# ming71/rotate-yolov3

Measured on AMD Instinct MI355X. Metric: images/sec fwd+bwd at 608^2 (train step, backend=hip), higher is better.
Workload: dtype bf16; 1 GPU; configs[3]: Darknet-53 train step (fwd + riou loss + bwd + grad all-reduce + SGD), bs=64/GPU 608x608, synthetic HRSC-shaped targets; global_batch=64, parallelism=dp1, gradients=250 MB fp32 in 4 flat buckets, fp32 on the wire

## Files before the change

### include/ryolo.h

```cpp
#ifndef RYOLO_H
#define RYOLO_H

#include <stddef.h>
#include <stdint.h>

#ifdef __cplusplus
extern "C" {
#endif

#define RYOLO_OK 0
#define RYOLO_EINVAL -1
#define RYOLO_ELAUNCH -2
#define RYOLO_ETOOBIG -3

#define RYOLO_RNMS_MAX_BOXES 262144

const char *ryolo_strerror(int code);
int ryolo_abi_version(void);
const char *ryolo_build_id(void);
int ryolo_set_tuning(const char *name, const char *value);

size_t ryolo_rnms_workspace_bytes(int n);
int ryolo_rnms(const float *dets, int n, int row_stride, float thr, int64_t *keep_out, int32_t *num_keep,
               void *workspace, size_t workspace_bytes, void *stream);
// ... 49 lines not shown
#define RYOLO_CONV_KERNEL_STEM_DGRAD 7
#define RYOLO_CONV_KERNEL_STEM64 11
#define RYOLO_CONV_KERNEL_MQ128 9
#define RYOLO_CONV_KERNEL_MQ64 10
#define RYOLO_CONV_KERNEL_IGEMM 16
int ryolo_conv_kernel_choice(const ryolo_conv_desc *desc, int with_residual, int with_statistics);
#define RYOLO_WGRAD_KERNEL_TAPS 1000
int ryolo_conv_dgrad_kernel_choice(const ryolo_conv_desc *forward_desc, int with_bn_reduce );
int ryolo_conv_wgrad_kernel_choice(const ryolo_conv_desc *forward_desc);
int ryolo_nchw_f32_to_nhwc_bf16(const float *x, int N, int C, int H, int W, int Cpad, void *y, void *stream);
int ryolo_nhwc_bf16_to_nchw_f32(const void *x, int N, int C, int H, int W, int cstride, float *y, void *stream);


int ryolo_yolo_decode_filter(const void *head, int head_cstride, int bs, int ny, int nx, int na, int no,
                             const float *anchors, float stride, float context_factor, int arc, float conf_thres,
                             float min_wh, long long io_rows_per_image, long long io_row_offset, float *cand,
                             long long *cand_row, int *counter, int capacity, void *stream);

int ryolo_yolo_decode(const void *head, int head_cstride, int bs, int ny, int nx, int na, int no,
                      const float *anchors, float stride, float context_factor, int arc, float *io,
                      long long io_rows_per_image, long long io_row_offset, float *p, void *stream);

int ryolo_conv_head_decode_supported(const ryolo_conv_desc *desc, int na, int no);
int ryolo_conv_head_decode(const ryolo_conv_desc *desc, const void *x, const void *w_packed, const float *scale, const float *shift,
                           const float *anchors, int na, int no, float stride, float context_factor, int arc, float *io,
                           long long io_rows_per_image, long long io_row_offset, float *p, void *stream);

int ryolo_add_nhwc(const void *a, int a_cstride, const void *b, int b_cstride, void *y, int y_cstride,
                   long long npix, int C, void *stream);
int ryolo_upsample_nhwc(const void *x, int x_cstride, void *y, int y_cstride, int N, int H, int W, int C, int scale,
                        void *stream);
int ryolo_maxpool_nhwc(const void *x, int x_cstride, void *y, int y_cstride, int N, int H, int W, int C, int ksize,
                       int stride, void *stream);


int ryolo_conv0_recompute_supported(const ryolo_conv_desc *desc);
int ryolo_conv0_bn_act_fwd(const ryolo_conv_desc *desc, const void *x, const void *w_packed, const float *scale, const float *shift,
                           int act, const float *slope, void *y, void *stream);
size_t ryolo_conv0_bn_bwd_workspace_bytes(void);
int ryolo_conv0_bn_bwd(const ryolo_conv_desc *desc, const void *x, const void *w_packed, const void *dy, int dy_cstride,
                       const float *scale, const float *shift, const float *mean, const float *invstd, int act, const float *slope,
                       void *dz, int dz_cstride, float *dgamma, float *dbeta, float *dslope, void *workspace, size_t workspace_bytes,
                       int workspace_is_zero, void *stream);
size_t ryolo_conv0_bn_bwd_wgrad_workspace_bytes(void);
int ryolo_conv0_bn_bwd_wgrad(const ryolo_conv_desc *desc, const void *x, const void *w_packed, const void *dy, int dy_cstride,
                             const float *scale, const float *shift, const float *mean, const float *invstd, int act, const float *slope,
                             float *dgamma, float *dbeta, float *dslope, float *grad_oihw, int cin_real, int accumulate, void *workspace,
                             size_t workspace_bytes, void *stream);
int ryolo_conv_stat_rows(const ryolo_conv_desc *desc);
int ryolo_conv2d_bn_act_stats(const ryolo_conv_desc *desc, const void *x, const void *w_packed, const float *scale,
                              const float *shift, const void *residual, void *y,
                              double *stat_part ,
                              void *stream);
int ryolo_bn_finalize(double *stat_part, int rows, int cpad, int C, long long count, float eps, float momentum,
                      const float *gamma, const float *beta, float *mean, float *invstd, float *scale, float *shift,
                      float *running_mean , float *running_var, void *stream);
int ryolo_bn_act_fwd(const void *z, int z_cstride, const float *scale, const float *shift, int act,
                     const float *slope , const void *residual, int res_cstride, void *y,
                     int y_cstride, long long npix, int C, void *stream);
size_t ryolo_bn_act_bwd_workspace_bytes(long long npix, int C);
int ryolo_bn_act_bwd(const void *z, int z_cstride, const void *dy, int dy_cstride, const float *scale, const float *shift,
                     const float *mean, const float *invstd, int act, const float *slope, void *dz, int dz_cstride,
                     long long npix, int C, float *dgamma, float *dbeta, float *dslope, void *workspace,
                     size_t workspace_bytes, void *stream);
size_t ryolo_conv_packed_dgrad_bytes(int Cout, int Cin, int ksize, int stride);
int ryolo_conv_dgrad_tap_table(int ksize, int stride, int *host_out );
int ryolo_conv_pack_weights_dgrad(const float *w_oihw, int Cout, int Cin, int ksize, int stride, void *packed,
                                  const int *taps_table ,
                                  void *stream);
int ryolo_conv2d_dgrad(const ryolo_conv_desc *forward_desc, const void *dz, int dz_cstride, const void *packed_dgrad,
                       const float *ones, const float *zeros , void *dx, int accumulate, void *stream);
int ryolo_conv2d_dgrad_bnreduce_rows(const ryolo_conv_desc *forward_desc);
int ryolo_conv2d_dgrad_bnreduce(const ryolo_conv_desc *forward_desc, const void *dz, int dz_cstride, const void *packed_dgrad,
                                const float *ones, const float *zeros, void *dx, int accumulate,
                                const void *z , int z_cstride,
                                const float *scale, const float *shift, const float *mean, const float *invstd ,
                                const float *slope , float *part , void *stream);
int ryolo_bn_act_bwd_reduced(const void *z, int z_cstride, const void *dy, int dy_cstride, const float *scale, const float *shift,
                             const float *mean, const float *invstd, int act , const float *slope, void *dz,
                             int dz_cstride, long long npix, int C, float *dgamma, float *dbeta, float *dslope, const float *part,
                             int rows, void *workspace , size_t workspace_bytes, void *stream);
size_t ryolo_conv_wgrad_workspace_bytes(const ryolo_conv_desc *forward_desc);
int ryolo_conv2d_wgrad_partials(const ryolo_conv_desc *forward_desc, const void *x, const void *dz, int dz_cstride, int Cin_real,
                                float *grad_oihw, int accumulate, void *workspace, size_t workspace_bytes, void *stream);
int ryolo_conv2d_wgrad_reduce(const ryolo_conv_desc *forward_desc, const void *x, const void *dz, int dz_cstride, int Cin_real,
                              float *grad_oihw, int accumulate, void *workspace, size_t workspace_bytes, void *stream);

typedef struct ryolo_wgrad_reduce_job {
    const float *part;
    float *g;
    int S, Cout, Cin_real, Cin_k, ks, Kpad, Cout_pad, accumulate;
    int kind;
    int block_begin, block_end;
    int wide;
} ryolo_wgrad_reduce_job;
int ryolo_conv_wgrad_reduce_job_fill(ryolo_wgrad_reduce_job *host_job, const ryolo_conv_desc *forward_desc, int Cin_real, const void *workspace,
                                     float *grad_oihw, int accumulate);
int ryolo_conv_wgrad_reduce_batch(const ryolo_wgrad_reduce_job *device_jobs, int njobs, int total_blocks, void *stream);
int ryolo_conv2d_wgrad(const ryolo_conv_desc *forward_desc, const void *x, const void *dz, int dz_cstride, int Cin_real,
                       float *grad_oihw , int accumulate, void *workspace,
                       size_t workspace_bytes, void *stream);
int ryolo_upsample2x_bwd(const void *dy, int dy_cstride, void *dx, int dx_cstride, int N, int H, int W, int C,
                         int accumulate, void *stream);
int ryolo_pgrad_to_nhwc(const float *pgrad, int bs, int na, int ny, int nx, int no, void *out, int out_cstride,
                        void *stream);

typedef struct ryolo_pack_job {
    const void *src;
    void *dst;
    int kind, Cout, Cin, KS, Cin_pad, ntaps, Kpad, rows;
    int khs[9], kws[9];
    int block_begin, block_end;
// ... 57 lines not shown
```

### rotate-yolov3_amd/csrc/conv.hip

```cpp
#include <cstring>

#include <mutex>

#include "conv_common.h"

namespace ryolo_detail {
thread_local int *g_conv_choice = nullptr;
}

using namespace ryolo_detail;

namespace {

template <int KS, int BM, int BN, int WGM, int WGN, int NSTAGE, bool FAST, bool GEN, bool BNRED = false>
__global__ void __launch_bounds__(WGM *WGN * 64) conv_igemm_kernel(const ConvParams p, const BnRed br = BnRed()) {
    constexpr int NW = WGM * WGN, NT = NW * 64;
    constexpr int WPIX = BM / WGM, WCH = BN / WGN, PF = WPIX / 16, CF = WCH / 16;
    constexpr int A_BYTES = BM * BK * 2, B_BYTES = BN * BK * 2, STAGE = A_BYTES + B_BYTES;
    constexpr int A_PPW = (BM / 8) / NW, B_PPW = (BN / 8) / NW;
    static_assert(A_PPW >= 1 && B_PPW >= 1, "tile too small for the wave count");
    constexpr int SROW = BN * 2 + 16;
    static_assert(BM * SROW + WGM * 2 * BN * 4 <= NSTAGE * STAGE, "staging tile + statistics slots must fit in the operand buffers");
    constexpr int LOADS_PER_STAGE = A_PPW + B_PPW;

// ... 269 lines not shown
            const f32x4 sh = *(const f32x4 *)(p.shift + n0 + ch_local);
#pragma unroll
            for (int f = 0; f < PF; f++) {
                const int pix_local = wm * WPIX + f * 16 + frow;
                bf16x4 o;
#pragma unroll
                for (int r = 0; r < 4; r++) o[r] = (__bf16)actfn(acc[c][f][r] * sc[r] + sh[r]);
                *(bf16x4 *)(smem + pix_local * SROW + ch_local * 2) = o;
                if (GEN && p.stat_part) {
#pragma unroll
                    for (int r = 0; r < 4; r++) {
                        const float v = (float)o[r];
                        st_sum[c][r] += v;
                        st_sq[c][r] += v * v;
                    }
                }
            }
        }
    };
    const float slope = p.slope;
    if (p.act == RYOLO_ACT_LEAKY) epilogue1([slope](float v) { return v > 0.f ? v : v * slope; });
    else if (p.act == RYOLO_ACT_MISH) epilogue1([](float v) { return mish(v); });
    else epilogue1([](float v) { return v; });
    if (GEN && p.stat_part) {
        static_assert(CF <= 4, "one total per lane of a 16-lane row");
        float ta = 0.f, tb = 0.f;
#pragma unroll
        for (int c = 0; c < CF; c++)
#pragma unroll
            for (int r = 0; r < 4; r++) {
                const float a = row16_sum(st_sum[c][r]), b = row16_sum(st_sq[c][r]);
                if (frow == c * 4 + r) {
                    ta = a;
                    tb = b;
                }
            }
        float *slot = (float *)(smem + BM * SROW) + wm * 2 * BN;
        const int ch = wn * WCH + (frow >> 2) * 16 + fk * 4 + (frow & 3);
        if (frow < CF * 4) {
            slot[ch] = ta;
            slot[BN + ch] = tb;
        }
    }
    __syncthreads();
    if (GEN && p.stat_part) {
        static_assert(NT >= 2 * BN, "one thread per (statistic, channel)");
        if (tid < 2 * BN) {
            const float *slot = (const float *)(smem + BM * SROW);
            float v = slot[tid];
#pragma unroll
            for (int w = 1; w < WGM; w++) v += slot[w * 2 * BN + tid];
            const int st = tid / BN, ch = tid % BN;
            if (n0 + ch < p.Cout)
                atomicAdd(p.stat_part + (size_t)(m_tile % STAT_ROWS) * 2 * p.stat_cpad + (size_t)st * p.stat_cpad + n0 + ch, (double)v);
        }
    }

    constexpr int CPR = BN / 8;
    constexpr int NIT = BM * CPR / NT;
    static_assert(BM * CPR % NT == 0, "tile chunks must divide evenly over the threads");
    auto opix = [&](int m) -> size_t {
        int j, i, img;
        split_pixel(m, p.Wo, p.Ho, p.magic_wo, p.magic_ho, p.use_magic, j, i, img);
        return ((size_t)img * p.OH + (size_t)(i * p.os + p.ooy)) * p.OW + (size_t)(j * p.osx + p.oox);
    };
    bf16x8 rv[NIT];
    if (p.res) {
#pragma unroll
        for (int it = 0; it < NIT; it++) {
            const int idx = it * NT + tid;
            const int m = m0 + idx / CPR, c = n0 + (idx % CPR) * 8;
            const bool ok = (m < p.M) && (c < p.Cout);
            rv[it] = *(const bf16x8 *)(ok ? p.res + ((!GEN || p.os == 1) ? (size_t)m : opix(m)) * p.res_cs + c : zero_page);
        }
    }
    static_assert(!BNRED || (NT % CPR == 0 && CPR <= 16 && !GEN && CPR == BR_CPR && NIT == BR_NIT), "a thread keeps one 8-channel chunk for all its pixels");
    float bn_sc[8], bn_sh[8], bn_mu[8], bn_is[8], bs1[8], bs2[8], bs3[8];
    float bn_slope = 0.f;
    if constexpr (BNRED) {
        bn_slope = br.slope[0];
        const int c = n0 + (tid % CPR) * 8;
        const bool okc = c < p.Cout;
        const f32x4 z4 = f32x4{0.f, 0.f, 0.f, 0.f};
        const f32x4 a0 = okc ? *(const f32x4 *)(br.scale + c) : z4, a1 = okc ? *(const f32x4 *)(br.scale + c + 4) : z4;
        const f32x4 b0 = okc ? *(const f32x4 *)(br.shift + c) : z4, b1 = okc ? *(const f32x4 *)(br.shift + c + 4) : z4;
        const f32x4 u0 = okc ? *(const f32x4 *)(br.mean + c) : z4, u1 = okc ? *(const f32x4 *)(br.mean + c + 4) : z4;
        const f32x4 i0 = okc ? *(const f32x4 *)(br.invstd + c) : z4, i1 = okc ? *(const f32x4 *)(br.invstd + c + 4) : z4;
#pragma unroll
        for (int e = 0; e < 4; e++) {
            bn_sc[e] = a0[e]; bn_sc[4 + e] = a1[e]; bn_sh[e] = b0[e]; bn_sh[4 + e] = b1[e]; bn_mu[e] = u0[e]; bn_mu[4 + e] = u1[e];
            bn_is[e] = i0[e]; bn_is[4 + e] = i1[e];
        }
#pragma unroll
        for (int e = 0; e < 8; e++) bs1[e] = bs2[e] = bs3[e] = 0.f;
    }
#pragma unroll
    for (int it = 0; it < NIT; it++) {
        const int idx = it * NT + tid;
        const int pix = idx / CPR, ch = (idx % CPR) * 8;
        const int m = m0 + pix, c = n0 + ch;
        if (m >= p.M || c >= p.Cout) continue;
        bf16x8 v = *(const bf16x8 *)(smem + pix * SROW + ch * 2);
        if (p.res) {
#pragma unroll
            for (int e = 0; e < 8; e++) v[e] = (__bf16)((float)v[e] + (float)rv[it][e]);
        }
        if constexpr (BNRED) {
// ... 173 lines not shown

    const __bf16 *zero_page = p.w + (size_t)(((p.Cout + 127) >> 7) << 7) * p.Kpad;
    const int KT = p.Kpad / BK;
    const float slope = p.slope;
    f32x4 acc[CF][PF];

    int i = loc;
    setup(start + i);
    int m0 = nm0, n0 = nn0;
    int buf = 0;
    stage(0, buf, true);
    f32x4 ep_sc[CF], ep_sh[CF];
    auto load_scale_shift = [&]() {
#pragma unroll
        for (int c = 0; c < CF; c++) {
            const int ch_local = wn * WCH + c * 16 + fk * 4;
            ep_sc[c] = *(const f32x4 *)(p.scale + n0 + ch_local);
            ep_sh[c] = *(const f32x4 *)(p.shift + n0 + ch_local);
        }
    };
    load_scale_shift();
    float st_sum[CF][4], st_sq[CF][4];
#pragma unroll
    for (int c = 0; c < CF; c++)
#pragma unroll
        for (int r = 0; r < 4; r++) st_sum[c][r] = st_sq[c][r] = 0.f;
    auto flush_stats = [&]() {
        static_assert(!STATS || (CF <= 4 && NT >= 2 * BN), "one total per lane of a 16-lane row; one thread per (statistic, channel)");
        float ta = 0.f, tb = 0.f;
#pragma unroll
        for (int c = 0; c < CF; c++)
#pragma unroll
            for (int r = 0; r < 4; r++) {
                const float a = row16_sum(st_sum[c][r]), b = row16_sum(st_sq[c][r]);
                if (frow == c * 4 + r) {
                    ta = a;
                    tb = b;
                }
                st_sum[c][r] = st_sq[c][r] = 0.f;
            }
        float *slots = (float *)(smem + 2 * STAGE);
        const int ch = wn * WCH + (frow >> 2) * 16 + fk * 4 + (frow & 3);
        if (frow < CF * 4) {
            slots[wm * 2 * BN + ch] = ta;
            slots[wm * 2 * BN + BN + ch] = tb;
        }
        __syncthreads();
        if (tid < 2 * BN) {
            float v = slots[tid];
#pragma unroll
            for (int w = 1; w < WGM; w++) v += slots[w * 2 * BN + tid];
            const int st = tid / BN, c = tid % BN;
            if (n0 + c < p.Cout)
                atomicAdd(p.stat_part + ((size_t)(blockIdx.x % STAT_ROWS) * 2 + st) * p.stat_cpad + n0 + c, (double)v);
        }
        __syncthreads();
    };
    static_assert(!BNRED || (NT % CPR == 0 && CPR == 16 && !STATS), "a lane keeps one 8-channel chunk; 4 lanes of a wave share it");
    float bs1[8], bs2[8], bs3[8];
#pragma unroll
    for (int e = 0; e < 8; e++) bs1[e] = bs2[e] = bs3[e] = 0.f;
    const float bn_slope = BNRED ? br.slope[0] : 0.f;
    auto flush_bn = [&]() {
        if constexpr (BNRED) {
            const int cch = tid % CPR, c = n0 + cch * 8;
            float *slots = (float *)(smem + 2 * STAGE);
#pragma unroll
            for (int e = 0; e < 8; e++) {
                float a = bs1[e], b = bs2[e] * (c + e < p.Cout ? br.invstd[c + e] : 0.f), d = bs3[e];
                a += __shfl_xor(a, 16); b += __shfl_xor(b, 16); d += __shfl_xor(d, 16);
                a += __shfl_xor(a, 32); b += __shfl_xor(b, 32); d += __shfl_xor(d, 32);
                if (lane < CPR) {
                    slots[(wave * CPR + cch) * 24 + e] = a;
                    slots[(wave * CPR + cch) * 24 + 8 + e] = b;
                    slots[(wave * CPR + cch) * 24 + 16 + e] = d;
                }
                bs1[e] = bs2[e] = bs3[e] = 0.f;
            }
            __syncthreads();
            for (int t = tid; t < CPR * 24; t += NT) {
                const int l = t / 24, k = t % 24;
                float v = slots[l * 24 + k];
#pragma unroll
                for (int w = 1; w < NW; w++) v += slots[(w * CPR + l) * 24 + k];
                const int ch = n0 + l * 8 + (k & 7);
                if (ch < p.Cout) br.part[((size_t)blockIdx.x * 3 + (k >> 3)) * p.Cout + ch] += v;
            }
            __syncthreads();
        }
    };
    while (true) {
        const int inext = i + nloc;
        const bool has_next = inext < len;
#pragma unroll
        for (int c = 0; c < CF; c++)
#pragma unroll
            for (int f = 0; f < PF; f++) acc[c][f] = f32x4{0.f, 0.f, 0.f, 0.f};
        auto compute = [&](int cb) {
            const char *sb = smem + cb * STAGE;
#pragma unroll
            for (int ks = 0; ks < 2; ks++) {
                bf16x8 wf[CF], xf[PF];
#pragma unroll
                for (int c = 0; c < CF; c++) wf[c] = *(const bf16x8 *)(sb + b_off[c][ks]);
#pragma unroll
                for (int f = 0; f < PF; f++) xf[f] = *(const bf16x8 *)(sb + a_off[f][ks]);
#pragma unroll
// ... 324 lines not shown
    };
    u4 xa[3], xb[3];
    u2 da[2], db[2];
    request(xa, true);
    request_dy(da, m, true);
    for (int it = 0; it < n_it; it += 2) {
        const int m_a = m;
        advance();
        request(xb, it + 1 < n_it);
        request_dy(db, m, it + 1 < n_it);
        finish(xa, da, m_a, true);
        const int m_b = m;
        advance();
        request(xa, it + 2 < n_it);
        request_dy(da, m, it + 2 < n_it);
        finish(xb, db, m_b, it + 1 < n_it);
    }
    if constexpr (MODE == 2) {
        float t1 = 0.f, t2 = 0.f, t3 = 0.f;
#pragma unroll
        for (int cf = 0; cf < 2; cf++)
#pragma unroll
            for (int r = 0; r < 4; r++) {
                const float a1 = row16_sum(b1[cf][r]), a2 = row16_sum(b2[cf][r]), a3 = row16_sum(b3[cf][r]);
                if (fr == cf * 4 + r) {
                    t1 = a1;
                    t2 = a2;
                    t3 = a3;
                }
            }
        if (fr < 8) {
            const int ch = (fr >> 2) * 16 + g * 4 + (fr & 3);
            double *row = bw.part + (size_t)(wave_id % STAT_ROWS) * 3 * 32;
            atomicAdd(row + ch, (double)t1);
            atomicAdd(row + 32 + ch, (double)t2);
            atomicAdd(row + 64 + ch, (double)t3);
        }
        return;
    }
    if (STATS) {
        float ta = 0.f, tb = 0.f;
#pragma unroll
        for (int cf = 0; cf < 2; cf++)
#pragma unroll
            for (int r = 0; r < 4; r++) {
                const float a = row16_sum(st_sum[cf][r]), b = row16_sum(st_sq[cf][r]);
                if (fr == cf * 4 + r) {
                    ta = a;
                    tb = b;
                }
            }
        if (fr < 8) {
            const int ch = (fr >> 2) * 16 + g * 4 + (fr & 3);
            double *row = p.stat_part + (size_t)(wave_id % STAT_ROWS) * 2 * p.stat_cpad;
            atomicAdd(row + ch, (double)ta);
            atomicAdd(row + p.stat_cpad + ch, (double)tb);
        }
    }
}

__global__ void conv0_bwd_finalize_kernel(double *__restrict__ part, const float *__restrict__ scale, const float *__restrict__ mean,
                                          const float *__restrict__ invstd, float inv_count, float *__restrict__ kb, float *__restrict__ kd,
                                          float *__restrict__ dgamma, float *__restrict__ dbeta, float *__restrict__ dslope) {
    const int c = threadIdx.x;
    double a = 0.0, b = 0.0, d = 0.0;
    for (int r = 0; r < STAT_ROWS; r++) {
        double *row = part + (size_t)r * 96;
        a += row[c]; b += row[32 + c]; d += row[64 + c];
        row[c] = 0.0; row[32 + c] = 0.0; row[64 + c] = 0.0;
    }
    const float s1 = (float)a, s2 = (float)b * invstd[c];
    if (dgamma) dgamma[c] += s2;
    if (dbeta) dbeta[c] += s1;
    const float k = scale[c] * invstd[c] * s2 * inv_count;
    kb[c] = -k;
    kd[c] = k * mean[c] - scale[c] * s1 * inv_count;
    if (dslope) {
        float v = (float)d;
#pragma unroll
        for (int o = 16; o > 0; o >>= 1) v += __shfl_xor(v, o, 32);
        if (c == 0) dslope[0] += v;
    }
}

template <int ACT>
static int launch_c8_bwd(ConvParams &p, int gpw, unsigned nblk, const C8Bwd &bw, int mode, hipStream_t stream) {
    if (mode == 2) hipLaunchKernelGGL((conv3x3_c8_direct_kernel<false, ACT, 2>), dim3(nblk), dim3(256), 0, stream, p, gpw, bw);
    else hipLaunchKernelGGL((conv3x3_c8_direct_kernel<false, ACT, 3>), dim3(nblk), dim3(256), 0, stream, p, gpw, bw);
    return hipGetLastError() == hipSuccess ? RYOLO_OK : RYOLO_ELAUNCH;
}

template <bool STATS>
int launch_c8_direct(ConvParams &p, int gpw, unsigned nblk, hipStream_t stream) {
    if (STATS && p.y == nullptr) {
        hipLaunchKernelGGL((conv3x3_c8_direct_kernel<true, RYOLO_ACT_LINEAR, 1>), dim3(nblk), dim3(256), 0, stream, p, gpw, C8Bwd());
        return hipGetLastError() == hipSuccess ? RYOLO_OK : RYOLO_ELAUNCH;
    }
    if (p.act == RYOLO_ACT_LEAKY) hipLaunchKernelGGL((conv3x3_c8_direct_kernel<STATS, RYOLO_ACT_LEAKY>), dim3(nblk), dim3(256), 0, stream, p, gpw);
    else if (p.act == RYOLO_ACT_MISH) hipLaunchKernelGGL((conv3x3_c8_direct_kernel<STATS, RYOLO_ACT_MISH>), dim3(nblk), dim3(256), 0, stream, p, gpw);
    else hipLaunchKernelGGL((conv3x3_c8_direct_kernel<STATS, RYOLO_ACT_LINEAR>), dim3(nblk), dim3(256), 0, stream, p, gpw);
    return hipGetLastError() == hipSuccess ? RYOLO_OK : RYOLO_ELAUNCH;
}

__global__ void pack_weights_kernel(const float *__restrict__ w, int Cout, int Cin, int KS, int Cin_pad, int Kpad,
                                    int Cout_pad, __bf16 *__restrict__ out) {
    const size_t total = (size_t)Cout_pad * Kpad + 128;
    for (size_t i = (size_t)blockIdx.x * blockDim.x + threadIdx.x; i < total; i += (size_t)gridDim.x * blockDim.x) {
// ... 360 lines not shown
            if (pick == 1) pick = 7;
        }
    }
    if (pick == 8) return launch_conv_mp(p, 256, 0, stream);
    if (pick == 11) return launch_conv_mp(p, 192, 0, stream);
    if (pick == 14) return launch_conv_mp(p, 0, 0, stream);
    if (pick == 9) return launch_conv_mq(p, 0, stream);
#ifdef RYOLO_MP_ABLATION
    if (pick >= 32 && pick < 64) return launch_conv_mp(p, (pick & 16) ? 192 : 256, ryolo_mp_ablation_variant(pick & 15), stream);
    if (pick >= 64 && pick < 80) return launch_conv_mq(p, ryolo_mp_ablation_variant(pick & 15), stream);
#endif
    if (ksize == 1) {
        if (pick == 1) {
            const long long T = (((long long)p.M + 127) / 128) * ((p.Cout + 127) / 128);
            if (p.fast && p.os == 1 && !(p.stat_part && p.res) && !p.no_persist && (p.force_persist || 2 * T >= 5 * (long long)((2 * cu_count()) & ~7)))
                return launch_variant<1, 128, 128, 2, 2>(p, stream);
            p.no_persist = 1;
            return launch_variant<1, 128, 128, 2, 4>(p, stream);
        }
        if (pick == 7) return launch_variant<1, 128, 128, 2, 2>(p, stream);
        if (pick == 2) return launch_variant<1, 256, 64, 4, 1>(p, stream);
        if (pick == 3) return launch_variant<1, 256, 32, 4, 1>(p, stream);
        if (pick == 4) return launch_variant<1, 256, 128, 4, 2, 3>(p, stream);
        if (pick == 6) return launch_variant<1, 128, 128, 4, 2>(p, stream);
    } else {
        if (pick == 1) return launch_variant<3, 128, 128, 2, 4>(p, stream);
        if (pick == 7) return launch_variant<3, 128, 128, 2, 2>(p, stream);
        if (pick == 2) return launch_variant<3, 256, 64, 4, 1>(p, stream);
        if (pick == 3) return launch_variant<3, 256, 32, 4, 1>(p, stream);
        if (pick == 4) return launch_variant<3, 256, 128, 4, 2, 3>(p, stream);
        if (pick == 6) return launch_variant<3, 128, 128, 4, 2>(p, stream);
    }
    return RYOLO_EINVAL;
}

static int validate(const ryolo_conv_desc *d) {
    if (!d) return RYOLO_EINVAL;
    if (d->ksize != 1 && d->ksize != 3) return RYOLO_EINVAL;
    if (d->N <= 0 || d->H <= 0 || d->W <= 0 || d->Cin <= 0 || d->Cout <= 0 || d->stride <= 0) return RYOLO_EINVAL;
    if ((d->Cin & 7) || (d->Cout & 7) || (d->in_cstride & 7) || (d->out_cstride & 7)) return RYOLO_EINVAL;
    if (d->in_cstride < d->Cin || d->out_cstride < d->Cout) return RYOLO_EINVAL;
    if (d->upsample != 1 && d->upsample != 2) return RYOLO_EINVAL;
    if (d->ksize == 1 && d->pad != 0) return RYOLO_EINVAL;
    return RYOLO_OK;
}

int ryolo_conv_stat_rows(const ryolo_conv_desc *d) {
    if (validate(d) != RYOLO_OK) return 0;
    return STAT_ROWS;
}

int ryolo_conv2d_bn_act_stats(const ryolo_conv_desc *d, const void *x, const void *w_packed, const float *scale,
                              const float *shift, const void *residual, void *y, double *stat_part, void *stream_) {
    if (validate(d) != RYOLO_OK || !x || !w_packed || !scale || !shift) return RYOLO_EINVAL;
    if (!y && !(stat_part && ryolo_conv0_recompute_supported(d))) return RYOLO_EINVAL;
    if (residual && ((d->res_cstride & 7) || d->res_cstride < d->Cout)) return RYOLO_EINVAL;
    if (((uintptr_t)x | (uintptr_t)y | (uintptr_t)w_packed | (uintptr_t)residual | (uintptr_t)scale | (uintptr_t)shift) & 15)
        return RYOLO_EINVAL;
    ConvParams p;
    p.x = (const __bf16 *)x;
    p.w = (const __bf16 *)w_packed;
    p.scale = scale;
    p.shift = shift;
    p.res = (const __bf16 *)residual;
    p.y = (__bf16 *)y;
    p.N = d->N; p.H = d->H; p.W = d->W; p.Cin = d->Cin; p.in_cs = d->in_cstride;
    p.stride = d->stride;
    p.pad = d->pad;
    p.Ho = (d->H + 2 * d->pad - d->ksize) / d->stride + 1;
    p.Wo = (d->W + 2 * d->pad - d->ksize) / d->stride + 1;
    if (p.Ho <= 0 || p.Wo <= 0) return RYOLO_EINVAL;
    p.Cout = d->Cout; p.out_cs = d->out_cstride; p.res_cs = d->res_cstride;
    p.K = d->ksize * d->ksize * d->Cin;
    p.Kpad = (p.K + BK - 1) / BK * BK;
    const long long M = (long long)d->N * p.Ho * p.Wo;
    if (M > 0x7fffffffLL - 512) return RYOLO_EINVAL;
    p.M = (int)M;
    p.cin_log2 = ilog2_exact(d->Cin);
    if (d->ksize == 3 && p.cin_log2 < 0 && (d->Cin % BK)) return RYOLO_EINVAL;
    p.act = d->act; p.slope = d->slope; p.ups = d->upsample; p.nt = 0;
    {
        const unsigned long long xb = (((unsigned long long)d->N * d->H * d->W - 1) * d->in_cstride + d->Cin) * 2ull;
        const unsigned long long wb = ((unsigned long long)((d->Cout + 127) / 128 * 128) * p.Kpad + 128) * 2ull;
        p.taps2 = (d->Cin == 32 && d->ksize == 3) ? 1 : 0;
        p.fast = (d->Cin % BK == 0 || p.taps2) && xb < 0x7fffff00ull && wb < 0x7fffff00ull && !(d->tile & 0x100);
        if (!p.fast) p.taps2 = 0;
        p.x_bytes = (unsigned)(p.fast ? xb : 0);
        p.w_bytes = (unsigned)(p.fast ? wb : 0);
    }
    p.ntaps = d->ksize * d->ksize;
    for (int t = 0; t < 9; t++) { p.tap_dy[t] = t / d->ksize; p.tap_dx[t] = t % d->ksize; }
    p.os = 1; p.osx = 1; p.ooy = 0; p.oox = 0; p.OH = p.Ho; p.OW = p.Wo;
    p.no_persist = (d->tile & 0x200) ? 1 : 0;
    p.force_persist = (d->tile & 0x800) ? 1 : 0;
    p.pw_grid_cap = (d->tile & 0xff) == 13 ? (d->tile >> 16) & 0xff : 0;
#ifdef RYOLO_MP_ABLATION
    if ((d->tile & 0x400) && p.fast) p.x_bytes = p.w_bytes = 0;
#endif
    p.ntiles = 0; p.magic_wo = p.magic_ho = p.magic_nt = 0;
    p.nt_out = (long long)p.M * d->upsample * d->upsample * d->Cout * 2 >= nt_out_min_bytes() ? 1 : 0;
    p.stat_part = stat_part;
    p.stat_cpad = (d->Cout + 127) / 128 * 128;
    const unsigned long long c8_xb = (unsigned long long)d->N * d->H * d->W * 16ull, c8_yb = ((unsigned long long)(p.M - 1) * d->out_cstride + 32) * 2ull;
    if (d->ksize == 3 && d->stride == 1 && d->pad == 1 && d->Cin == 8 && d->in_cstride == 8 && d->Cout == 32 &&
        !residual && d->upsample == 1 && !(d->tile & 0x1ff) && p.Wo >= 16 && c8_xb < 0x7fffff00ull && c8_yb < 0x7fffff00ull) {
        p.x_bytes = (unsigned)c8_xb;
        p.w_bytes = (unsigned)c8_yb;
        const long long groups = ((long long)p.M + 15) / 16;
        const int gpw = (d->tile >> 16) ? (d->tile >> 16) : 32;
        const long long waves = (groups + gpw - 1) / gpw;
        const unsigned nblk = (unsigned)((waves + 3) / 4);
        const bool staged = conv0_halo_on() && !(d->tile >> 16) && y && !stat_part;
        RYOLO_CONV_DRY_RUN((staged ? RYOLO_CONV_KERNEL_STEM0 : RYOLO_CONV_KERNEL_DIRECT8));
        if (staged) return launch_conv0_halo(p, nullptr, 0, cu_count(), (hipStream_t)stream_);
        return stat_part ? launch_c8_direct<true>(p, gpw, nblk, (hipStream_t)stream_) : launch_c8_direct<false>(p, gpw, nblk, (hipStream_t)stream_);
    }
    return dispatch(p, d->ksize, pick_tile(d, d->Cout), (hipStream_t)stream_);
}

static bool head_params(const ryolo_conv_desc *d, ConvParams &p) {
    if (validate(d) != RYOLO_OK || d->ksize != 1 || d->stride != 1 || d->pad != 0 || d->upsample != 1 || (d->Cin % BK)) return false;
    p.N = d->N; p.H = d->H; p.W = d->W; p.Cin = d->Cin; p.in_cs = d->in_cstride; p.stride = 1; p.pad = 0; p.Ho = d->H; p.Wo = d->W;
    p.Cout = d->Cout; p.out_cs = d->Cout; p.res_cs = 0; p.K = d->Cin; p.Kpad = d->Cin;
    const long long M = (long long)d->N * d->H * d->W;
    if (M > 0x7fffffffLL - 512) return false;
    p.M = (int)M;
    p.act = d->act; p.slope = d->slope; p.ups = 1; p.nt = 0; p.taps2 = 0; p.os = 1; p.osx = 1; p.ooy = 0; p.oox = 0; p.OH = p.Ho; p.OW = p.Wo;
    const unsigned long long xb = (((unsigned long long)M - 1) * d->in_cstride + d->Cin) * 2ull;
    const unsigned long long wb = ((unsigned long long)((d->Cout + 127) / 128 * 128) * p.Kpad + 128) * 2ull;
    if (xb >= 0x7fffff00ull || wb >= 0x7fffff00ull) return false;
    p.fast = 1; p.x_bytes = (unsigned)xb; p.w_bytes = (unsigned)wb;
    p.res = nullptr; p.y = nullptr; p.stat_part = nullptr; p.stat_cpad = 0; p.nt_out = 0; p.pw_grid_cap = 0;
    p.no_persist = 0; p.force_persist = 0; p.ntaps = 1; p.ntiles = 0; p.magic_wo = p.magic_ho = p.magic_nt = 0; p.use_magic = 1;
    return true;
}

int ryolo_conv_head_decode_supported(const ryolo_conv_desc *d, int na, int no) {
    ConvParams p;
    return head_params(d, p) && conv_pw_decode_supported(p, na, no) ? 1 : 0;
}

int ryolo_conv_head_decode(const ryolo_conv_desc *d, const void *x, const void *w_packed, const float *scale, const float *shift,
                           const float *anchors, int na, int no, float stride, float context_factor, int arc, float *io,
                           long long io_rows_per_image, long long io_row_offset, float *pout, void *stream_) {
    ConvParams p;
    if (!x || !w_packed || !scale || !shift || !anchors || !io || !head_params(d, p) || !conv_pw_decode_supported(p, na, no)) return RYOLO_EINVAL;
    if (arc < 0 || arc > 2 || !(stride > 0.f) || !(context_factor > 0.f)) return RYOLO_EINVAL;
    if (((uintptr_t)x | (uintptr_t)w_packed) & 15) return RYOLO_EINVAL;
    p.x = (const __bf16 *)x; p.w = (const __bf16 *)w_packed; p.scale = scale; p.shift = shift;
    return launch_conv_pw_decode(p, io, io_rows_per_image, io_row_offset, pout, anchors, na, no, stride, context_factor, arc, (hipStream_t)stream_);
}

int ryolo_conv_pair_supported(const ryolo_conv_desc *first, const ryolo_conv_desc *second, int shortcut_from_input) {
    if (validate(first) != RYOLO_OK || validate(second) != RYOLO_OK) return 0;
    return conv_stem_pair_kind(first, second, shortcut_from_input) != 0 ? 1 : 0;
// ... 702 lines not shown
```

### rotate-yolov3_amd/csrc/conv_common.h

```cpp
#pragma once
#include <hip/hip_runtime.h>
#include <stdint.h>
#include <stdlib.h>

#include "../../include/ryolo.h"

namespace ryolo_detail {

typedef __attribute__((ext_vector_type(8))) __bf16 bf16x8;
typedef __attribute__((ext_vector_type(4))) __bf16 bf16x4;
typedef __attribute__((ext_vector_type(2))) __bf16 bf16x2;
typedef __attribute__((ext_vector_type(4))) float f32x4;
typedef __attribute__((ext_vector_type(4))) unsigned int u32x4;
typedef __attribute__((address_space(3))) void *lds_vp;
typedef const __attribute__((address_space(1))) void *glb_vp;

constexpr int BK = 64;
constexpr long long NT_OUT_MIN_BYTES = 128ll << 20;
constexpr int STAT_ROWS = 128;

struct ConvParams {
    const __bf16 *x;
    const __bf16 *w;
    const float *scale;
    const float *shift;
    const __bf16 *res;
    __bf16 *y;
    int N, H, W, Cin, in_cs;
    int Ho, Wo, Cout, out_cs, res_cs;
    int stride, pad;
    int K, Kpad, M;
    int cin_log2;
    int act;
    float slope;
    int ups;
    int nt;
    unsigned x_bytes, w_bytes;
    int fast;
    int taps2;
    int no_persist;
    int force_persist;
    int ntaps;
    int tap_dy[9], tap_dx[9];
    int os, ooy, oox, OH, OW;
    int osx;
    int ntiles;
    unsigned magic_wo, magic_ho, magic_nt;
    int use_magic;
    unsigned y_bytes, res_bytes;
    double *stat_part;
    int stat_cpad;
    int nt_out;
    int reg3;
    int korder = 0;
    int dbg0, dbg1;
    int pw_nb, pw_mb;
    unsigned *trace;
    int pw_grid_cap;
};

struct BnRed {
    const __bf16 *z;
    int z_cs;
    const float *scale, *shift, *mean, *invstd;
    const float *slope;
    float *part;
    unsigned z_bytes = 0;
};

__device__ __forceinline__ float mish(float v) {
    const float e = __expf(fminf(v, 20.f));
    const float n = (1.f + e) * (1.f + e);
    return v * (n - 1.f) / (n + 1.f);
}

__device__ __forceinline__ float row16_sum(float v) {
#if defined(__HIP_DEVICE_COMPILE__)
    v += __builtin_bit_cast(float, __builtin_amdgcn_update_dpp(0, __builtin_bit_cast(int, v), 0xB1, 0xF, 0xF, true));
    v += __builtin_bit_cast(float, __builtin_amdgcn_update_dpp(0, __builtin_bit_cast(int, v), 0x4E, 0xF, 0xF, true));
    v += __builtin_bit_cast(float, __builtin_amdgcn_update_dpp(0, __builtin_bit_cast(int, v), 0x141, 0xF, 0xF, true));
    v += __builtin_bit_cast(float, __builtin_amdgcn_update_dpp(0, __builtin_bit_cast(int, v), 0x140, 0xF, 0xF, true));
#endif
    return v;
}

template <int O>
__device__ __forceinline__ float lane_xor_sum(float v) {
#if defined(__HIP_DEVICE_COMPILE__)
    if constexpr (O == 4) {
        v += __builtin_bit_cast(float, __builtin_amdgcn_update_dpp(0, __builtin_bit_cast(int, v), 0x124, 0xF, 0xF, true));
    } else if constexpr (O == 8) {
        v += __builtin_bit_cast(float, __builtin_amdgcn_update_dpp(0, __builtin_bit_cast(int, v), 0x128, 0xF, 0xF, true));
    } else if constexpr (O == 16) {
        const unsigned u = __builtin_bit_cast(unsigned, v);
        const auto s = __builtin_amdgcn_permlane16_swap(u, u, false, false);
        v = __builtin_bit_cast(float, (unsigned)s[0]) + __builtin_bit_cast(float, (unsigned)s[1]);
    } else {
        static_assert(O == 32, "partner distance");
        const unsigned u = __builtin_bit_cast(unsigned, v);
        const auto s = __builtin_amdgcn_permlane32_swap(u, u, false, false);
        v = __builtin_bit_cast(float, (unsigned)s[0]) + __builtin_bit_cast(float, (unsigned)s[1]);
    }
#endif
    return v;
// ... 92 lines not shown
```

### rotate-yolov3_amd/csrc/conv_mp.hip

```cpp
#include <cstdlib>
#include <type_traits>

#include "conv_common.h"

using namespace ryolo_detail;

namespace {

constexpr int MP_BN = 256;
constexpr int MP_XB = 256 * 128, MP_WB = 256 * 128;
constexpr int MP_OPS = 2 * MP_XB + 2 * MP_WB;
constexpr int MP_SS = 2 * 2 * MP_BN * 4;
constexpr int MP_TRACE = 8 * 128 * 4;
constexpr int MP_LDS = MP_OPS + MP_SS + MP_TRACE;
constexpr int MP_STAT_NT = 4;
constexpr int MP_STAT = MP_STAT_NT * 2 * 2 * MP_BN * 4;
constexpr int MP_LDS_GEN = MP_LDS + MP_STAT;

template <int N> using ic = std::integral_constant<int, N>;

template <int BM, int GEN, int VAR, int KO = 0>
__global__ void __launch_bounds__(512) conv_mp_kernel(const ConvParams p) {
    constexpr int OPS = MP_OPS;
    constexpr int WBASE = 2 * MP_XB, XBASE = 0;
// ... 381 lines not shown
                    unsigned R[2][2];
#pragma unroll
                    for (int cc = 0; cc < 2; cc++) {
                        const int c = 2 * h + cc;
                        bf16x4 o;
#pragma unroll
                        for (int r = 0; r < 4; r++) {
                            float v = acc[c][f][r] * sc[cc][r] + sh[cc][r];
                            if constexpr (ACT == RYOLO_ACT_LEAKY) v = v > 0.f ? v : v * slope;
                            else if constexpr (ACT == 3) v = fmaxf(v, v * slope);
                            else if constexpr (ACT == RYOLO_ACT_MISH) v = mish(v);
                            o[r] = (__bf16)v;
                            if (GEN == 1 && p.stat_part && ok) {
                                const float q = (float)o[r];
                                st_sum[cc][r] += q;
                                st_sq[cc][r] += q * q;
                            }
                        }
                        const uint2 u = __builtin_bit_cast(uint2, o);
                        R[cc][0] = u.x;
                        R[cc][1] = u.y;
                    }
#if defined(__HIP_DEVICE_COMPILE__)
#pragma unroll
                    for (int d = 0; d < 2; d++) {
                        auto s1 = __builtin_amdgcn_permlane32_swap(R[0][d], R[1][d], false, false);
                        auto s2 = __builtin_amdgcn_permlane16_swap(s1[0], s1[1], false, false);
                        R[0][d] = s2[0];
                        R[1][d] = s2[1];
                    }
#endif
                    u32x4 out = u32x4{R[0][0], R[0][1], R[1][0], R[1][1]};
                    if (has_res) {
                        bf16x8 a = __builtin_bit_cast(bf16x8, out);
                        const bf16x8 b = __builtin_bit_cast(bf16x8, rv[f][h]);
#pragma unroll
                        for (int e = 0; e < 8; e++) a[e] = (__bf16)((float)a[e] + (float)b[e]);
                        out = __builtin_bit_cast(u32x4, a);
                    }
                    if constexpr (NO_STORE) {
                        asm volatile("" ::"v"(out.x), "v"(out.y), "v"(out.z), "v"(out.w));
                    } else {
                        int voff = yoff0, soff = f * ystep;
                        if (strided) { voff = (opix(ok ? m : 0) * p.out_cs + chq + fk * 8) * 2; soff = 0; }
                        voff = ok ? voff : (int)0x80000000;
#if defined(__HIP_DEVICE_COMPILE__)
                        if (STAUX == 0 && p.nt_out) buffer_store16_soff<2>(out, yrs, voff + 64 * h, soff);
                        else buffer_store16_soff<STAUX>(out, yrs, voff + 64 * h, soff);
#endif
                    }
                }
                stamp_e(3 + h);
                if (GEN == 1 && p.stat_part) {
                    double *row = p.stat_part + (size_t)(((m0 / BM) * 2 + wm) % STAT_ROWS) * 2 * p.stat_cpad;
                    float *slot = stat_lds + ((size_t)((n0 / MP_BN) * 2 + wm) * 2) * MP_BN + wn * 64;
                    float ta = 0.f, tb = 0.f;
#pragma unroll
                    for (int cc = 0; cc < 2; cc++)
#pragma unroll
                        for (int r = 0; r < 4; r++) {
                            const float a = row16_sum(st_sum[cc][r]), b = row16_sum(st_sq[cc][r]);
                            if (frow == cc * 4 + r) {
                                ta = a;
                                tb = b;
                            }
                        }
                    if (frow < 8) {
                        const int cl = (2 * h + (frow >> 2)) * 16 + fr4 + (frow & 3);
                        if (stat_in_lds) {
                            slot[cl] += ta;
                            slot[MP_BN + cl] += tb;
                        } else {
                            atomicAdd(row + chq + cl, (double)ta);
                            atomicAdd(row + p.stat_cpad + chq + cl, (double)tb);
                        }
                    }
                }
            }
          };
          if (p.act == RYOLO_ACT_LEAKY && p.slope <= 1.f) run_epilogue(ic<3>{});
          else if (p.act == RYOLO_ACT_LEAKY) run_epilogue(ic<RYOLO_ACT_LEAKY>{});
          else if (p.act == RYOLO_ACT_MISH) run_epilogue(ic<RYOLO_ACT_MISH>{});
          else run_epilogue(ic<RYOLO_ACT_LINEAR>{});
          ss[(sslot ^ 1) * (2 * MP_BN) + tid] = ss_next;
        }
        stamp_e(5);
        te_tile++;
        __builtin_amdgcn_sched_barrier(0);
        if (!has_next) break;
        sslot = __builtin_amdgcn_readfirstlane(sslot ^ 1);
        ti = tnext;
        m0 = nm0;
        n0 = nn0;
    }
    if constexpr (STAGGER) {
        if (wm == 0) __builtin_amdgcn_s_barrier();
    }
    if constexpr (GEN == 1) {
        if (stat_in_lds) {
            asm volatile("s_waitcnt lgkmcnt(0)" ::: "memory");
            __builtin_amdgcn_s_barrier();
            double *row = p.stat_part + (size_t)(blockIdx.x % STAT_ROWS) * 2 * p.stat_cpad;
            for (int i = tid; i < p.nt * 2 * MP_BN; i += 512) {
                const int s_ = i / (2 * MP_BN), st = (i / MP_BN) & 1, ch = i % MP_BN;
                const float *q = stat_lds + ((size_t)(s_ * 2) * 2 + st) * MP_BN + ch;
                const float v = q[0] + q[2 * MP_BN];
                if (v != 0.f && s_ * MP_BN + ch < p.Cout) atomicAdd(row + (size_t)st * p.stat_cpad + s_ * MP_BN + ch, (double)v);
            }
        }
    }
    asm volatile("s_waitcnt vmcnt(0)" ::: "memory");
    if constexpr (TRACE_EPI) {
        if ((blockIdx.x == 0 || blockIdx.x == 8 || blockIdx.x == 129) && p.stat_part) {
            asm volatile("s_waitcnt lgkmcnt(0)" ::: "memory");
            unsigned *dst = (unsigned *)p.stat_part + ((blockIdx.x == 0 ? 0 : (blockIdx.x == 8 ? 1 : 2)) * 8 + wave) * 32;
            if (lane < 32) dst[lane] = *(const unsigned *)(smem + trace_off + lane * 4);
        }
    }
}

inline unsigned mp_magic_u32(int d) { return d <= 1 ? 0u : (unsigned)((0x100000000ull + (unsigned)d - 1) / (unsigned)d); }

inline int mp_cu_count() {
    static int cus = 0;
    if (!cus) {
        int dev = 0;
        if (hipGetDevice(&dev) != hipSuccess ||
            hipDeviceGetAttribute(&cus, hipDeviceAttributeMultiprocessorCount, dev) != hipSuccess || cus <= 0)
            cus = 256;
    }
    return cus;
}

void *g_trace_buf = nullptr;
int g_dbg[4] = {0, 0, 0, 0};
int g_var[16] = {0};

template <int BM, int GEN, int VAR, int KO = 0>
int mp_launch(ConvParams &p, hipStream_t stream) {
    if (VAR & (128 | 1024)) p.stat_part = (double *)g_trace_buf;
    static bool attr_done = false;
    constexpr int LDS = GEN == 1 ? MP_LDS_GEN : MP_LDS;
    auto kfn = conv_mp_kernel<BM, GEN, VAR, KO>;
    if (!attr_done && !g_conv_choice) {
        if (hipFuncSetAttribute((const void *)kfn, hipFuncAttributeMaxDynamicSharedMemorySize, LDS) != hipSuccess)
            return RYOLO_ELAUNCH;
        attr_done = true;
    }
    const int mt = (p.M + BM - 1) / BM;
    p.nt = (p.Cout + MP_BN - 1) / MP_BN;
    const long long T = (long long)mt * p.nt;
    const long long dmax = p.Wo > p.Ho ? p.Wo : p.Ho, mpad = (long long)mt * BM;
    if (mpad * dmax >= 0x100000000ll || T * p.nt >= 0x100000000ll || T > 0x7fffffffll) return RYOLO_EINVAL;
    p.use_magic = 1;
    p.magic_wo = mp_magic_u32(p.Wo);
// ... 83 lines not shown
```

### rotate-yolov3_amd/csrc/conv_mq.hip

```cpp
#include <cstdlib>
#include <type_traits>

#include "conv_common.h"

using namespace ryolo_detail;

namespace {

#ifdef RYOLO_MP_ABLATION
constexpr int Q_TRACE = 4 * 128 * 4;
#else
constexpr int Q_TRACE = 0;
#endif
template <int CW, int PF>
struct QL {
    static constexpr int BN = 4 * CW;
    static constexpr int BM = 16 * PF;
    static constexpr int XB = BM * 128;
    static constexpr int WB = BN * 128;
    static constexpr int XBASE = 0, WBASE = 2 * XB;
    static constexpr int OPS = 2 * XB + WB;
    static constexpr int SS = 2 * 2 * BN * 4;
    static constexpr int LDS = OPS + SS + Q_TRACE;
    static constexpr int STAT_NT = CW == 64 ? 4 : 8;
// ... 431 lines not shown
                        auto s2 = __builtin_amdgcn_permlane16_swap(s1[0], s1[1], false, false);
                        R[0][d] = s2[0];
                        R[1][d] = s2[1];
                    }
#endif
                    u32x4 out = u32x4{R[0][0], R[0][1], R[1][0], R[1][1]};
                    if (has_res) {
                        bf16x8 a = __builtin_bit_cast(bf16x8, out);
                        const bf16x8 b = __builtin_bit_cast(bf16x8, rv[f][h]);
#pragma unroll
                        for (int e = 0; e < 8; e++) a[e] = (__bf16)((float)a[e] + (float)b[e]);
                        out = __builtin_bit_cast(u32x4, a);
                    }
                    if constexpr (BNRED) {
                        const bf16x8 a = __builtin_bit_cast(bf16x8, out), zb = __builtin_bit_cast(bf16x8, zv[f][h]);
#pragma unroll
                        for (int e = 0; e < 8; e++) {
                            const float zf = (float)zb[e], d = ok ? (float)a[e] : 0.f;
                            const float u = zf * bn_sc[e] + bn_sh[e];
                            float g = d;
                            if (u <= 0.f) { g = d * bn_slope; bs3[e] += d * u; }
                            bs2[e] += g * (zf - bn_mu[e]);
                            bs1[e] += g;
                        }
                    }
                    if constexpr (NO_STORE) {
                        asm volatile("" ::"v"(out.x), "v"(out.y), "v"(out.z), "v"(out.w));
                    } else {
                        int voff = yoff0, soff = f * ystep;
                        if (strided) { voff = (opix(ok ? m : 0) * p.out_cs + chq + fk * 8) * 2; soff = 0; }
                        voff = ok ? voff : (int)0x80000000;
#if defined(__HIP_DEVICE_COMPILE__)
                        if (p.nt_out) buffer_store16_soff<2>(out, yrs, voff + 64 * h, soff);
                        else buffer_store16_soff<0>(out, yrs, voff + 64 * h, soff);
#endif
                    }
                }
                stamp_e(3 + h);
                if constexpr (BNRED) {
                    float t1 = 0.f, t2 = 0.f, t3 = 0.f;
#pragma unroll
                    for (int e = 0; e < 8; e++) {
                        const float a = row16_sum(bs1[e]), b = row16_sum(bs2[e]), c = row16_sum(bs3[e]);
                        if (frow == e) { t1 = a; t2 = b; t3 = c; }
                    }
                    if (frow < 8) {
                        float *slot = stat_lds + (size_t)(n0 / Q_BN) * 3 * Q_BN + wn * CW + 32 * h + fk * 8 + frow;
                        slot[0] += t1;
                        slot[Q_BN] += t2;
                        slot[2 * Q_BN] += t3;
                    }
                }
                if (GEN == 1 && p.stat_part) {
                    double *row = p.stat_part + (size_t)((m0 / L::BM) % STAT_ROWS) * 2 * p.stat_cpad;
                    float *slot = stat_lds + (size_t)(n0 / Q_BN) * 2 * Q_BN + wn * CW;
                    float ta = 0.f, tb = 0.f;
#pragma unroll
                    for (int cc = 0; cc < 2; cc++)
#pragma unroll
                        for (int r = 0; r < 4; r++) {
                            const float a = row16_sum(st_sum[cc][r]), b = row16_sum(st_sq[cc][r]);
                            if (frow == cc * 4 + r) {
                                ta = a;
                                tb = b;
                            }
                        }
                    if (frow < 8) {
                        const int cl = (2 * h + (frow >> 2)) * 16 + fr4 + (frow & 3);
                        if (stat_in_lds) {
                            slot[cl] += ta;
                            slot[Q_BN + cl] += tb;
                        } else {
                            atomicAdd(row + chq + cl, (double)ta);
                            atomicAdd(row + p.stat_cpad + chq + cl, (double)tb);
                        }
                    }
                }
            }
          };
          if (p.act == RYOLO_ACT_LEAKY && p.slope <= 1.f) run_epilogue(ic<3>{});
          else if (p.act == RYOLO_ACT_LEAKY) run_epilogue(ic<RYOLO_ACT_LEAKY>{});
          else if (p.act == RYOLO_ACT_MISH) run_epilogue(ic<RYOLO_ACT_MISH>{});
          else run_epilogue(ic<RYOLO_ACT_LINEAR>{});
          ss[(sslot ^ 1) * (2 * Q_BN) + sst] = ssn0;
          ss[(sslot ^ 1) * (2 * Q_BN) + Q_BN + sst] = ssn1;
        }
        stamp_e(5);
        te_tile++;
        __builtin_amdgcn_sched_barrier(0);
        if (!has_next) break;
        sslot = __builtin_amdgcn_readfirstlane(sslot ^ 1);
        ti = tnext;
        m0 = nm0;
        n0 = nn0;
    }
    if constexpr (GEN == 1) {
        if (stat_in_lds) {
            asm volatile("s_waitcnt lgkmcnt(0)" ::: "memory");
            __builtin_amdgcn_s_barrier();
            double *row = p.stat_part + (size_t)(blockIdx.x % STAT_ROWS) * 2 * p.stat_cpad;
            for (int i = tid; i < p.nt * 2 * Q_BN; i += 256) {
                const int s_ = i / (2 * Q_BN), st = (i / Q_BN) & 1, ch = i % Q_BN;
                const float v = stat_lds[(size_t)(s_ * 2 + st) * Q_BN + ch];
                if (v != 0.f && s_ * Q_BN + ch < p.Cout) atomicAdd(row + (size_t)st * p.stat_cpad + s_ * Q_BN + ch, (double)v);
            }
        }
    }
    if constexpr (BNRED) {
        asm volatile("s_waitcnt lgkmcnt(0)" ::: "memory");
        __builtin_amdgcn_s_barrier();
        for (int i = tid; i < p.nt * 3 * Q_BN; i += 256) {
            const int s_ = i / (3 * Q_BN), k3 = (i / Q_BN) % 3, ch = s_ * Q_BN + i % Q_BN;
            if (ch < p.Cout) {
                float v = stat_lds[i];
                if (k3 == 1) v *= br.invstd[ch];
                br.part[((size_t)blockIdx.x * 3 + k3) * p.Cout + ch] = v;
            }
        }
    }
    asm volatile("s_waitcnt vmcnt(0)" ::: "memory");
    if constexpr (TRACE_EPI) {
        if ((blockIdx.x == 0 || blockIdx.x == 256 || blockIdx.x == 8) && p.stat_part) {
            asm volatile("s_waitcnt lgkmcnt(0)" ::: "memory");
            unsigned *dst = (unsigned *)p.stat_part + ((blockIdx.x == 0 ? 0 : (blockIdx.x == 256 ? 1 : 2)) * 8 + wn) * 32;
            if (lane < 32) dst[lane] = *(const unsigned *)(smem + trace_off + lane * 4);
        }
    }
}

inline unsigned mq_magic_u32(int d) { return d <= 1 ? 0u : (unsigned)((0x100000000ull + (unsigned)d - 1) / (unsigned)d); }

inline int mq_cu_count() {
    static int cus = 0;
    if (!cus) {
        int dev = 0;
        if (hipGetDevice(&dev) != hipSuccess ||
            hipDeviceGetAttribute(&cus, hipDeviceAttributeMultiprocessorCount, dev) != hipSuccess || cus <= 0)
            cus = 256;
    }
    return cus;
}

#ifdef RYOLO_MP_ABLATION
void *g_q_trace_buf = nullptr;
int g_q_dbg[4] = {0, 0, 0, 0};
#endif

inline int mq_grid_for(long long T, int cw = 64) {
    int per_cu = 2;
    if (cw == 32) {
        const char *e = abl_env("RYOLO_MQ128_WGPC");
        const int v = e ? atoi(e) : 2;
        if (v >= 1 && v <= 4) per_cu = v;
// ... 143 lines not shown
```

### rotate-yolov3_amd/csrc/conv_pw.hip

```cpp
#include <type_traits>
#include <utility>

#include "conv_common.h"
#include "yolo_decode.h"

using namespace ryolo_detail;

namespace {

template <int N> using ic = std::integral_constant<int, N>;

template <class F, int... I>
__device__ __forceinline__ void static_for_impl(F &&f, std::integer_sequence<int, I...>) {
    (f(ic<I>{}), ...);
}
template <int N, class F>
__device__ __forceinline__ void static_for(F &&f) {
    static_for_impl(f, std::make_integer_sequence<int, N>{});
}

__device__ __forceinline__ void issue_order_fence() { asm volatile("" ::: "memory"); }

template <int N>
__device__ __forceinline__ void wait_vmcnt() {
// ... 355 lines not shown
                if (PW_DBG(3)) {
                    asm volatile("" ::"v"(out));
                } else if (p.ups == 1) {
                    const int voff = ok ? (m * p.out_cs + och) * 2 : (int)0x80000000;
                    if (p.nt_out) __builtin_amdgcn_raw_buffer_store_b128(out, yrs, voff, 0, 2);
                    else __builtin_amdgcn_raw_buffer_store_b128(out, yrs, voff, 0, 0);
                } else {
                    const int mm = m < p.M ? m : 0;
                    const int t = udiv_magic(mm, p.magic_wo);
                    const int wo = mm - t * p.Wo;
                    const int img = udiv_magic(t, p.magic_ho);
                    const int ho = t - img * p.Ho;
                    const int W2 = p.Wo * 2;
                    const int o00 = ok ? ((((img * p.Ho * 2 + ho * 2) * W2 + wo * 2) * p.out_cs) + och) * 2 : (int)0x80000000;
                    buffer_store16_soff<0>(out, yrs, o00, 0);
                    buffer_store16_soff<0>(out, yrs, o00, p.out_cs * 2);
                    buffer_store16_soff<0>(out, yrs, o00, W2 * p.out_cs * 2);
                    buffer_store16_soff<0>(out, yrs, o00, (W2 + 1) * p.out_cs * 2);
                }
            }
#endif
        };
        if (p.act == RYOLO_ACT_LEAKY) run_epilogue(ic<RYOLO_ACT_LEAKY>{});
        else if (p.act == RYOLO_ACT_MISH) run_epilogue(ic<RYOLO_ACT_MISH>{});
        else run_epilogue(ic<RYOLO_ACT_LINEAR>{});
        PW_STAMP();
    };
    PW_STAMP();
    if (PW_DBG(7)) {
        asm volatile("s_waitcnt vmcnt(0)" ::: "memory");
        return;
    }
    row_block(0, ic<1>{});
    if (!PW_DBG(8))
        for (int i = 1; i < cnt; i++) row_block(i, ic<0>{});
    asm volatile("s_waitcnt vmcnt(0)" ::: "memory");
    PW_STAMP();

    if constexpr (STATS) {
        float ta = 0.f, tb = 0.f;
#pragma unroll
        for (int cf = 0; cf < CF; cf++)
#pragma unroll
            for (int rr = 0; rr < 4; rr++) {
                const float a = row16_sum(st_sum[cf][rr]), b = row16_sum(st_sq[cf][rr]);
                if (fr == cf * 4 + rr) {
                    ta = a;
                    tb = b;
                }
            }
        if (fr < CF * 4) {
            const int ch = n0 + wave * CF * 16 + (fr >> 2) * 16 + g * 4 + (fr & 3);
            if (ch < p.Cout) {
                double *row = p.stat_part + (size_t)(blockIdx.x % STAT_ROWS) * 2 * p.stat_cpad;
                atomicAdd(row + ch, (double)ta);
                atomicAdd(row + p.stat_cpad + ch, (double)tb);
            }
        }
    }
    if constexpr (BNRED) {
        float t1 = 0.f, t2 = 0.f, t3 = 0.f;
#pragma unroll
        for (int e = 0; e < 8; e++) {
            float a = row16_sum(bs1[e]), b = row16_sum(bs2[e]), d = row16_sum(bs3[e]);
            if constexpr (CF == 1) {
                a += __shfl_xor(a, 16); b += __shfl_xor(b, 16); d += __shfl_xor(d, 16);
            }
            if (fr == e) { t1 = a; t2 = b; t3 = d; }
        }
        const bool writer = fr < 8 && (CF == 2 || (g & 1) == 0);
        const int ch = och + fr;
        if (writer && ch < p.Cout) {
            float *row = br.part + (size_t)blockIdx.x * 3 * p.Cout;
            row[ch] = t1;
            row[p.Cout + ch] = t2 * br.invstd[ch];
            row[2 * p.Cout + ch] = t3;
        }
    }
}

struct PwCfg { int kt, ncb, nw, cf, pf, ring; };

static thread_local const PwDecode *g_pw_decode = nullptr;

template <int KT, int NW, int CF, int PF, int RING, int MODE>
int pw_launch(ConvParams &p, const PwBnRed &br, int grid, hipStream_t stream) {
    constexpr int LDS = RING * PF * 16 * 128 + (MODE == 4 ? PF * 16 * (NW * CF * 16 * 2 + 16) : 0);
    static bool attr_done = false;
    auto kfn = conv_pw_kernel<KT, NW, CF, PF, RING, MODE>;
    if (!attr_done) {
        if (LDS > 64 * 1024 && hipFuncSetAttribute((const void *)kfn, hipFuncAttributeMaxDynamicSharedMemorySize, LDS) != hipSuccess)
            return RYOLO_ELAUNCH;
        attr_done = true;
    }
    const PwDecode dc = g_pw_decode ? *g_pw_decode : PwDecode{};
    hipLaunchKernelGGL(kfn, dim3((unsigned)grid), dim3(NW * 64), LDS, stream, p, br, dc);
    return hipGetLastError() == hipSuccess ? RYOLO_OK : RYOLO_ELAUNCH;
}

template <int KT, int NW, int CF, int PF, int RING, int MODES>
int pw_launch_mode(ConvParams &p, const PwBnRed *br, int grid, hipStream_t stream) {
    PwBnRed none{};
    const int mode = g_pw_decode ? 4 : (br ? 3 : (p.stat_part ? 1 : (p.res ? 2 : 0)));
    if constexpr ((MODES & 16) != 0) if (mode == 4) return pw_launch<KT, NW, CF, PF, RING, 4>(p, none, grid, stream);
    if constexpr ((MODES & 8) != 0) if (mode == 3) return pw_launch<KT, NW, CF, PF, RING, 3>(p, *br, grid, stream);
    if constexpr ((MODES & 2) != 0) if (mode == 1) return pw_launch<KT, NW, CF, PF, RING, 1>(p, none, grid, stream);
    if constexpr ((MODES & 4) != 0) if (mode == 2) return pw_launch<KT, NW, CF, PF, RING, 2>(p, none, grid, stream);
// ... 179 lines not shown
```

### rotate-yolov3_amd/csrc/conv_stem.hip

```cpp
#include <type_traits>

#include "conv_common.h"

namespace ryolo_detail {
namespace {

template <int N> using ic = std::integral_constant<int, N>;

constexpr int TW = 32;
constexpr int CIN = 32, COUT = 64, CG = COUT / 16;

template <int S>
struct Patch {
    static constexpr int TH = S == 1 ? 8 : 4;
    static constexpr int PH = (TH - 1) * S + 3, PW = (TW - 1) * S + 3, NPIX = PH * PW;
    static constexpr int NPIECE = (NPIX + 15) / 16;
    static constexpr int PPW = (NPIECE + 3) / 4;
    static constexpr int BUF = PPW * 4 * 1024;
    static constexpr int BYTES = 2 * BUF;
    static constexpr int GPW = TH * TW / 16 / 4;
};

__device__ __forceinline__ int chunk_swz(int pcol) { return (pcol ^ (pcol >> 2)) & 3; }

// ... 111 lines not shown
                o2[cg][0] = u.x;
                o2[cg][1] = u.y;
            }
#pragma unroll
            for (int h = 0; h < CG / 2; h++) {
#if defined(__HIP_DEVICE_COMPILE__)
#pragma unroll
                for (int d = 0; d < 2; d++) {
                    auto sw = __builtin_amdgcn_permlane16_swap(o2[2 * h][d], o2[2 * h + 1][d], false, false);
                    o2[2 * h][d] = sw[0];
                    o2[2 * h + 1][d] = sw[1];
                }
#endif
                u32x4 outv = u32x4{o2[2 * h][0], o2[2 * h][1], o2[2 * h + 1][0], o2[2 * h + 1][1]};
                if constexpr (!STATS) {
                    if (p.res) {
                        bf16x8 ov = __builtin_bit_cast(bf16x8, outv);
#pragma unroll
                        for (int e = 0; e < 8; e++) ov[e] = (__bf16)((float)ov[e] + (float)rv[h][e]);
                        outv = __builtin_bit_cast(u32x4, ov);
                    }
                }
                if (ok) {
                    u32x4 *dst = (u32x4 *)(p.y + m * p.out_cs + h * 32 + run0);
                    if (p.nt_out) __builtin_nontemporal_store(outv, dst);
                    else *dst = outv;
                }
            }
        }
    }
    if constexpr (STATS) {
        float ta = 0.f, tb = 0.f;
#pragma unroll
        for (int cg = 0; cg < CG; cg++)
#pragma unroll
            for (int rr = 0; rr < 4; rr++) {
                const float a = row16_sum(st_sum[cg][rr]), b = row16_sum(st_sq[cg][rr]);
                if (fr == cg * 4 + rr) {
                    ta = a;
                    tb = b;
                }
            }
        __syncthreads();
        float *slots = (float *)smem;
        const int ch = (fr >> 2) * 16 + g * 4 + (fr & 3);
        slots[(wave * 2 + 0) * COUT + ch] = ta;
        slots[(wave * 2 + 1) * COUT + ch] = tb;
        __syncthreads();
        if (tid < 2 * COUT) {
            const int st = tid / COUT, c = tid % COUT;
            float v = slots[st * COUT + c];
#pragma unroll
            for (int w = 1; w < 4; w++) v += slots[(w * 2 + st) * COUT + c];
            atomicAdd(p.stat_part + ((size_t)(blockIdx.x % STAT_ROWS) * 2 + st) * p.stat_cpad + c, (double)v);
        }
    }
}

constexpr int C0_TH = 8, C0_TW = 64, C0_PH = C0_TH + 2, C0_PW = C0_TW + 2, C0_NPIX = C0_PH * C0_PW;
constexpr int C0_NPIECE = (C0_NPIX + 63) / 64;
constexpr int C0_PPW = (C0_NPIECE + 3) / 4, C0_BUF = C0_PPW * 4 * 1024;

template <int ACT>
__global__ void __launch_bounds__(256) conv0_halo_kernel(const ConvParams p, const float *slope_dev, int round_z, int tiles_x, int tiles_y, int ntiles) {
    extern __shared__ __attribute__((aligned(16))) char smem[];
    typedef __attribute__((ext_vector_type(4))) unsigned int u4;
    const int tid = threadIdx.x, lane = tid & 63;
    const int wave = __builtin_amdgcn_readfirstlane(tid >> 6);
    const int fr = lane & 15, g = lane >> 4;
    const int q8 = ntiles >> 3, r8 = ntiles & 7, xcd = blockIdx.x & 7, loc = blockIdx.x >> 3, nloc = gridDim.x >> 3;
    const int start = xcd < r8 ? xcd * (q8 + 1) : r8 * (q8 + 1) + (xcd - r8) * q8;
    const int len = q8 + (xcd < r8 ? 1 : 0);
    bf16x8 wfr[2][3];
#pragma unroll
    for (int cf = 0; cf < 2; cf++)
#pragma unroll
        for (int ks = 0; ks < 3; ks++) wfr[cf][ks] = *(const bf16x8 *)(p.w + (size_t)(cf * 16 + fr) * p.Kpad + ks * 32 + g * 8);
    f32x4 sc[2], sh[2];
#pragma unroll
    for (int cf = 0; cf < 2; cf++) {
        sc[cf] = *(const f32x4 *)(p.scale + cf * 16 + g * 4);
        sh[cf] = *(const f32x4 *)(p.shift + cf * 16 + g * 4);
    }
    const float slope = slope_dev ? slope_dev[0] : p.slope;
    int rel[3];
    bool tok[3];
#pragma unroll
    for (int ks = 0; ks < 3; ks++) {
        const int tap = ks * 4 + g, kh = (tap * 11) >> 5, kw = tap - 3 * kh;
        tok[ks] = tap < 9;
        rel[ks] = tok[ks] ? ((kh * C0_PW + kw) + fr) * 16 : 0;
    }
    const int tiles_img = tiles_x * tiles_y;
    auto fill = [&](int id, char *buf) {
        const int img = id / tiles_img, rem = id - img * tiles_img;
        const int ty = rem / tiles_x, tx = rem - ty * tiles_x;
        const int h0 = ty * C0_TH - 1, w0 = tx * C0_TW - 1;
#pragma unroll
        for (int j = 0; j < C0_PPW; j++) {
            const int piece = wave * C0_PPW + j;
            const int q = piece * 64 + lane;
            const int prow = q / C0_PW, pcol = q - prow * C0_PW;
            const int hi = h0 + prow, wi = w0 + pcol;
            const bool ok = q < C0_NPIX && (unsigned)hi < (unsigned)p.H && (unsigned)wi < (unsigned)p.W;
            const int off = ((img * p.H + hi) * p.W + wi) * 16;
            buffer_load_lds16(p.x, p.x_bytes, buf + piece * 1024, ok ? off : (int)0x80000000, 0);
        }
// ... 526 lines not shown
                        }
                    } else {
#pragma unroll
                        for (int rr = 0; rr < 4; rr++) {
                            float v = acc[u][cg][rr] * sc[cg][rr] + sh[cg][rr];
                            if constexpr (ACT == RYOLO_ACT_LEAKY) v = v > 0.f ? v : v * slope;
                            else if constexpr (ACT == RYOLO_ACT_MISH) v = mish(v);
                            o[rr] = (__bf16)v;
                        }
                    }
                    const uint2 uu = __builtin_bit_cast(uint2, o);
                    o2[cg][0] = uu.x;
                    o2[cg][1] = uu.y;
                }
#if defined(__HIP_DEVICE_COMPILE__)
#pragma unroll
                for (int d = 0; d < 2; d++) {
                    auto sw = __builtin_amdgcn_permlane16_swap(o2[0][d], o2[1][d], false, false);
                    o2[0][d] = sw[0];
                    o2[1][d] = sw[1];
                }
#endif
                u32x4 outv = u32x4{o2[0][0], o2[0][1], o2[1][0], o2[1][1]};
                if constexpr (!STATS) {
                    if (p.res) {
                        bf16x8 ov = __builtin_bit_cast(bf16x8, outv);
#pragma unroll
                        for (int e = 0; e < 8; e++) ov[e] = (__bf16)((float)ov[e] + (float)rv[u][e]);
                        outv = __builtin_bit_cast(u32x4, ov);
                    }
                }
                if (ok_[u]) {
                    u32x4 *dst = (u32x4 *)(p.y + (mbase + u * 16) * p.out_cs + co0 + run0);
                    if (p.nt_out) __builtin_nontemporal_store(outv, dst);
                    else *dst = outv;
                }
            }
        }
    }
    if constexpr (STATS) {
        float ta = 0.f, tb = 0.f;
#pragma unroll
        for (int cg = 0; cg < 2; cg++)
#pragma unroll
            for (int rr = 0; rr < 4; rr++) {
                const float a = row16_sum(st_sum[cg][rr]), b = row16_sum(st_sq[cg][rr]);
                if (fr == cg * 4 + rr) {
                    ta = a;
                    tb = b;
                }
            }
        if (fr < 8) {
            const int ch = co0 + (fr >> 2) * 16 + g * 4 + (fr & 3);
            double *row = p.stat_part + (size_t)(blockIdx.x % STAT_ROWS) * 2 * p.stat_cpad;
            atomicAdd(row + ch, (double)ta);
            atomicAdd(row + p.stat_cpad + ch, (double)tb);
        }
    }
}

template <bool STATS, int ACT>
int launch_stem64(ConvParams &p, int grid, int tiles_x, int tiles_y, int ntiles, hipStream_t stream) {
    hipLaunchKernelGGL((conv3x3_c64_halo_kernel<STATS, ACT>), dim3((unsigned)grid), dim3(256), c64::BYTES, stream, p, tiles_x, tiles_y, ntiles);
    return hipGetLastError() == hipSuccess ? RYOLO_OK : RYOLO_ELAUNCH;
}

template <int S, bool STATS>
int launch_stem(ConvParams &p, int grid, int tiles_x, int tiles_y, int ntiles, hipStream_t stream) {
    constexpr int smem = Patch<S>::BYTES;
    static bool attr_done = false;
    if (!attr_done) {
        if (smem > 64 * 1024 && hipFuncSetAttribute((const void *)conv3x3_c32_halo_kernel<S, STATS>,
                                                    hipFuncAttributeMaxDynamicSharedMemorySize, smem) != hipSuccess)
            return RYOLO_ELAUNCH;
        attr_done = true;
    }
    hipLaunchKernelGGL((conv3x3_c32_halo_kernel<S, STATS>), dim3((unsigned)grid), dim3(256), smem, stream, p, tiles_x, tiles_y, ntiles);
    return hipGetLastError() == hipSuccess ? RYOLO_OK : RYOLO_ELAUNCH;
}

}

bool conv_stem_eligible(const ConvParams &p, int ksize) {
    return ksize == 3 && p.Cin == CIN && p.Cout == COUT && p.pad == 1 && (p.stride == 1 || p.stride == 2) && p.fast && p.os == 1 &&
           p.ups == 1 && p.ntaps == 9 && (p.in_cs & 7) == 0 && (p.out_cs & 7) == 0 && (!p.res || (p.res_cs & 7) == 0) &&
           !(p.stat_part && p.res) && (long long)p.N * p.H * p.W * p.in_cs * 2 < 0x7fffff00ll;
}

bool conv_stem64_eligible(const ConvParams &p, int ksize) {
    return ksize == 3 && p.Cin == c64::CIN && p.Cout == c64::COUT && p.pad == 1 && p.stride == 1 && p.fast && p.os == 1 &&
           p.ups == 1 && p.ntaps == 9 && (p.in_cs & 7) == 0 && (p.out_cs & 7) == 0 && (!p.res || (p.res_cs & 7) == 0) &&
           !(p.stat_part && p.res) && (long long)p.N * p.H * p.W * p.in_cs * 2 < 0x7fffff00ll;
}

int launch_conv_stem64(ConvParams &p, int cus, hipStream_t stream) {
    const int tiles_x = (p.Wo + c64::TWX - 1) / c64::TWX, tiles_y = (p.Ho + c64::TH - 1) / c64::TH;
    const long long nt = (long long)p.N * tiles_x * tiles_y;
    if (nt > 0x7fffffffll) return RYOLO_EINVAL;
    RYOLO_CONV_DRY_RUN(RYOLO_CONV_KERNEL_STEM64);
    int grid = (2 * cus) & ~7;
    if (grid < 8) grid = 8;
    if (p.stat_part) return launch_stem64<true, RYOLO_ACT_LINEAR>(p, grid, tiles_x, tiles_y, (int)nt, stream);
    if (p.act == RYOLO_ACT_LEAKY) return launch_stem64<false, RYOLO_ACT_LEAKY>(p, grid, tiles_x, tiles_y, (int)nt, stream);
    if (p.act == RYOLO_ACT_MISH) return launch_stem64<false, RYOLO_ACT_MISH>(p, grid, tiles_x, tiles_y, (int)nt, stream);
    return launch_stem64<false, RYOLO_ACT_LINEAR>(p, grid, tiles_x, tiles_y, (int)nt, stream);
}

// ... 203 lines not shown
```

### rotate-yolov3_amd/csrc/rnms.hip

```cpp
#include <hip/hip_runtime.h>
#include <hipcub/hipcub.hpp>
#include <stdint.h>

#include <mutex>

#include "../../include/ryolo.h"
#include "conv_common.h"

#pragma clang fp contract(off)

namespace {

constexpr int WAVE = 64;
constexpr int MAX_PTS = 24;
constexpr int FAST_PTS = 8;

__device__ __forceinline__ void sincosf_cr(float a, float &s_out, float &c_out) {
    double x = (double)a;
    if (!(fabs(x) <= 1.0e6)) {
        if (!(fabs(x) <= 3.5e38)) {
            s_out = (float)(x - x);
            c_out = (float)(x - x);
            return;
        }
// ... 773 lines not shown
    const dim3 grid((unsigned)((kj + MASK_WAVES - 1) / MASK_WAVES), (unsigned)(row_hi - row_lo), (unsigned)num_segments);
    if (ct == 2)
        hipLaunchKernelGGL(rnms_mask_multi_kernel<2>, grid, dim3(MASK_WAVES * WAVE), 0, stream, n, thr, P0, P1, AUX, tiles, summ, seg_off,
                           seg_tile_stride, g_pair_counter, thr < 0.f ? 0 : 1, row_lo);
    else
        hipLaunchKernelGGL(rnms_mask_multi_kernel<1>, grid, dim3(MASK_WAVES * WAVE), 0, stream, n, thr, P0, P1, AUX, tiles, summ, seg_off,
                           seg_tile_stride, g_pair_counter, thr < 0.f ? 0 : 1, row_lo);
}

struct SidePool {
    hipStream_t s = nullptr;
    hipEvent_t a = nullptr, b = nullptr;
    int state = 0;
};
static std::mutex g_side_mutex;
static SidePool g_side[16];
static SidePool *side_pool() {
    int dev = 0;
    if (hipGetDevice(&dev) != hipSuccess || dev < 0 || dev >= 16) { (void)hipGetLastError(); return nullptr; }
    SidePool &sp = g_side[dev];
    if (sp.state == 0) {
        const bool ok = hipStreamCreateWithFlags(&sp.s, hipStreamNonBlocking) == hipSuccess &&
                        hipEventCreateWithFlags(&sp.a, hipEventDisableTiming) == hipSuccess &&
                        hipEventCreateWithFlags(&sp.b, hipEventDisableTiming) == hipSuccess;
        if (!ok) {
            (void)hipGetLastError();
            if (sp.b) (void)hipEventDestroy(sp.b);
            if (sp.a) (void)hipEventDestroy(sp.a);
            if (sp.s) (void)hipStreamDestroy(sp.s);
            sp.s = nullptr;
            sp.a = sp.b = nullptr;
            (void)hipGetLastError();
        }
        sp.state = ok ? 1 : -1;
    }
    return sp.state == 1 ? &sp : nullptr;
}
constexpr int SPLIT_MIN_ROWS = 320;

}

extern "C" {

const char *ryolo_strerror(int code) {
    switch (code) {
        case RYOLO_OK: return "ok";
        case RYOLO_EINVAL: return "invalid argument";
        case RYOLO_ELAUNCH: return "HIP launch failed (no gfx950 device, or a previous asynchronous error)";
        case RYOLO_ETOOBIG: return "too many boxes for one rotated-NMS call";
        default: return "unknown ryolo error";
    }
}

int ryolo_abi_version(void) { return 3; }

void ryolo_rnms_count_pairs(uint64_t *device_counter) { g_pair_counter = (unsigned long long *)device_counter; }


size_t ryolo_rnms_workspace_bytes(int n) {
    if (n <= 0) return 256;
    if (n > RYOLO_RNMS_MAX_BOXES) return 0;
    return rnms_layout(n).total;
}

int ryolo_rnms(const float *dets, int n, int row_stride, float thr, int64_t *keep_out, int32_t *num_keep,
               void *workspace, size_t workspace_bytes, void *stream_) {
    hipStream_t stream = (hipStream_t)stream_;
    if (n < 0 || !num_keep) return RYOLO_EINVAL;
    if (n == 0) {
        return hipMemsetAsync(num_keep, 0, sizeof(int32_t), stream) == hipSuccess ? RYOLO_OK : RYOLO_ELAUNCH;
    }
    if (!dets || !keep_out || !workspace || row_stride < 6) return RYOLO_EINVAL;
    if (n > RYOLO_RNMS_MAX_BOXES) return RYOLO_ETOOBIG;
    const RnmsLayout L = rnms_layout(n);
    if (workspace_bytes < L.total) return RYOLO_EINVAL;
    char *ws = (char *)workspace;
    uint32_t *keys_in = (uint32_t *)(ws + L.keys_in), *keys_out = (uint32_t *)(ws + L.keys_out);
    int32_t *idx_in = (int32_t *)(ws + L.idx_in), *order = (int32_t *)(ws + L.order);
    float4 *P0 = (float4 *)(ws + L.p0), *P1 = (float4 *)(ws + L.p1), *AUX = (float4 *)(ws + L.aux);
    uint4 *summ = (uint4 *)(ws + L.summ);
    unsigned char *flags = (unsigned char *)(ws + L.flags);
    unsigned long long *tiles = (unsigned long long *)(ws + L.tiles);

    const int tb = 256, nb = (n + tb - 1) / tb;
    hipLaunchKernelGGL(rnms_keys_kernel, dim3(nb), dim3(tb), 0, stream, dets, n, row_stride, keys_in, idx_in);
    size_t cub_bytes = L.cub_bytes;
    if (hipcub::DeviceRadixSort::SortPairs(ws + L.cub, cub_bytes, keys_in, keys_out, idx_in, order, n, 0, 32,
                                           stream) != hipSuccess)
        return RYOLO_ELAUNCH;
    uint32_t *ext = (uint32_t *)(ws + L.ext);
    if (hipMemsetAsync(ext, 0, 8 * sizeof(uint32_t), stream) != hipSuccess) return RYOLO_ELAUNCH;
    hipLaunchKernelGGL(rnms_extent_kernel, dim3(nb < 32 ? nb : 32), dim3(tb), 0, stream, dets, n, row_stride, ext);
    hipLaunchKernelGGL(rnms_corners_kernel, dim3(nb), dim3(tb), 0, stream, dets, n, row_stride, order, ext, P0, P1, AUX);
    const int W = (n + WAVE - 1) / WAVE;
    const size_t smem = scan_smem_bytes(W);
    scan_allow_big_lds();
    unsigned long long *state = (unsigned long long *)(ws + L.state);
    bool split = W >= SPLIT_MIN_ROWS;
    {
        const char *e = ryolo_detail::abl_env("RYOLO_RNMS_SPLIT");
        if (e && e[0] == '0') split = false;
    }
    if (split) {
        hipStreamCaptureStatus cs = hipStreamCaptureStatusNone;
        if (hipStreamIsCapturing(stream, &cs) != hipSuccess) { (void)hipGetLastError(); split = false; }
        else if (cs != hipStreamCaptureStatusNone) split = false;
    }
// ... 94 lines not shown
```

### rotate-yolov3_amd/csrc/train.hip

```cpp
#include <hip/hip_runtime.h>
#include <stdint.h>
#include <stdlib.h>

#include "../../include/ryolo.h"

namespace {

typedef __attribute__((ext_vector_type(8))) __bf16 bf16x8;
typedef __attribute__((ext_vector_type(4))) float f32x4;
typedef __attribute__((address_space(3))) void *lds_vp;
typedef short s16x4 __attribute__((ext_vector_type(4)));
typedef short s16x8 __attribute__((ext_vector_type(8)));

__device__ __forceinline__ s16x4 lds_read_tr16(const char *addr) {
#if defined(__HIP_DEVICE_COMPILE__)
    return __builtin_amdgcn_ds_read_tr16_b64_v4i16((__attribute__((address_space(3))) s16x4 *)(addr));
#else
    return s16x4{0, 0, 0, 0};
#endif
}

template <int T>
__device__ __forceinline__ int wg_swz(int row) {
    if (T >= 128) return (row & 3) | (((row >> 3) & 1) << 2);
// ... 759 lines not shown
        const unsigned unit = bid * R + r;
        glb_f32 dst = (glb_f32)(g_ + (size_t)unit * 576);
#pragma unroll
        for (int k = 0; k < 3; k++) {
            const int j = threadIdx.x + 256 * k;
            gv[r][k] = (accumulate && unit < nunits && j < 576) ? dst[j] : 0.f;
        }
    }
#pragma unroll
    for (int r = 0; r < R; r++) {
        const unsigned unit = bid * R + r;
        glb_f32 dst = (glb_f32)(g_ + (size_t)unit * 576);
#pragma unroll
        for (int k = 0; k < 3; k++) {
            const int j = threadIdx.x + 256 * k;
            const int cl = j / 9, tap = j - cl * 9;
            if (unit < nunits && j < 576) {
                const float v = sm[r * 9 * 65 + tap * 65 + cl];
                dst[j] = accumulate ? gv[r][k] + v : v;
            }
        }
    }
}
__host__ __device__ inline int wgrad_reduce_t3v_units_per_block(int S) { return S <= 3 ? 4 : 2; }
__device__ __forceinline__ void wgrad_reduce_t3v_body(float *sm, unsigned bid, const float *__restrict__ part, int S, int Cout, int Cin, int Cin_k,
                                                      int Kpad, int Cout_pad, float *__restrict__ g_, int accumulate, int wide) {
    if (!wide) wgrad_reduce_t3v_units<7, 1>(sm, bid, part, S, Cout, Cin, Cin_k, Kpad, Cout_pad, g_, accumulate);
    else if (S <= 3) wgrad_reduce_t3v_units<3, 4>(sm, bid, part, S, Cout, Cin, Cin_k, Kpad, Cout_pad, g_, accumulate);
    else wgrad_reduce_t3v_units<7, 2>(sm, bid, part, S, Cout, Cin, Cin_k, Kpad, Cout_pad, g_, accumulate);
}

__global__ void __launch_bounds__(256) wgrad_reduce_batch_kernel(const ryolo_wgrad_reduce_job *__restrict__ jobs, int njobs) {
    __shared__ __attribute__((aligned(16))) float sm[4096];
    int lo = 0;
    if (njobs <= 256) {
        lo = __syncthreads_count((int)threadIdx.x < njobs && jobs[threadIdx.x].block_begin <= (int)blockIdx.x) - 1;
    } else {
        int hi = njobs - 1;
        while (lo < hi) {
            const int mid = (lo + hi + 1) >> 1;
            if (jobs[mid].block_begin <= (int)blockIdx.x) lo = mid; else hi = mid - 1;
        }
    }
    lo = __builtin_amdgcn_readfirstlane(lo);
    const ryolo_wgrad_reduce_job j = jobs[lo];
    const unsigned bid = (unsigned)((int)blockIdx.x - j.block_begin), nblk = (unsigned)(j.block_end - j.block_begin);
    if (j.kind == 3) wgrad_reduce_v4_body(sm, bid, nblk, j.part, j.S, j.Cout, j.Cin_real, j.Cin_k, j.ks, j.Kpad, j.Cout_pad, j.g, j.accumulate, j.wide);
    else if (j.kind == 4) wgrad_reduce_t3v_body(sm, bid, j.part, j.S, j.Cout, j.Cin_real, j.Cin_k, j.Kpad, j.Cout_pad, j.g, j.accumulate, j.wide);
    else if (j.kind == 2) wgrad_reduce_t3_body(sm, bid, j.part, j.S, j.Cin_real, j.Cin_k, j.Kpad, j.Cout_pad, j.g, j.accumulate);
    else if (j.kind == 1) wgrad_reduce_body<4>(sm, bid, nblk, j.part, j.S, j.Cout, j.Cin_real, j.Cin_k, j.ks, j.Kpad, j.Cout_pad, j.g, j.accumulate);
    else wgrad_reduce_body<1>(sm, bid, nblk, j.part, j.S, j.Cout, j.Cin_real, j.Cin_k, j.ks, j.Kpad, j.Cout_pad, j.g, j.accumulate);
}

__global__ void __launch_bounds__(1024) bn_finalize_kernel(double *__restrict__ part, int R, int cpad, int C, float count, float eps,
                                   float momentum, const float *__restrict__ gamma, const float *__restrict__ beta,
                                   float *__restrict__ mean, float *__restrict__ invstd, float *__restrict__ scale,
                                   float *__restrict__ shift, float *__restrict__ run_mean, float *__restrict__ run_var) {
    __shared__ double red[2][32][33];
    const int cx = threadIdx.x & 31, ry = threadIdx.x >> 5;
    const int c = blockIdx.x * 32 + cx;
    double s = 0.0, q = 0.0;
    if (c < C) {
        for (int r0 = ry; r0 < R; r0 += 32 * 8) {
            double a[8], b[8];
#pragma unroll
            for (int u = 0; u < 8; u++) {
                const int r = r0 + 32 * u;
                a[u] = r < R ? part[(size_t)r * 2 * cpad + c] : 0.0;
                b[u] = r < R ? part[(size_t)r * 2 * cpad + cpad + c] : 0.0;
            }
#pragma unroll
            for (int u = 0; u < 8; u++) {
                const int r = r0 + 32 * u;
                s += a[u];
                q += b[u];
                if (r < R) {
                    part[(size_t)r * 2 * cpad + c] = 0.0;
                    part[(size_t)r * 2 * cpad + cpad + c] = 0.0;
                }
            }
        }
    }
    red[0][ry][cx] = s;
    red[1][ry][cx] = q;
    __syncthreads();
    if (ry != 0 || c >= C) return;
    for (int k = 1; k < 32; k++) { s += red[0][k][cx]; q += red[1][k][cx]; }
    const double mu = s / count;
    double var = q / count - mu * mu;
    if (var < 0) var = 0;
    const float is = (float)(1.0 / sqrt(var + (double)eps));
    mean[c] = (float)mu;
    invstd[c] = is;
    scale[c] = gamma[c] * is;
    shift[c] = beta[c] - (float)mu * gamma[c] * is;
    if (run_mean) {
        const double unb = count > 1.f ? var * count / (count - 1.0) : var;
        run_mean[c] = (1.f - momentum) * run_mean[c] + momentum * (float)mu;
        run_var[c] = (1.f - momentum) * run_var[c] + momentum * (float)unb;
    }
}

__device__ __forceinline__ float mish_f(float x) {
    const float e = __expf(fminf(x, 20.f));
    const float n = (1.f + e) * (1.f + e);
    return x * (n - 1.f) / (n + 1.f);
}
__device__ __forceinline__ float mish_grad(float x) {
    const float e = __expf(fminf(x, 20.f));
    const float n = (1.f + e) * (1.f + e);
    const float t = (n - 1.f) / (n + 1.f);
    return t + x * (1.f - t * t) * (e / (1.f + e));
}

constexpr long long NT_MIN_BYTES = 128ll << 20;
#ifdef RYOLO_MP_ABLATION
static int g_nt[3] = {-1, -1, -1};
inline bool nt_pass(int kind, long long npix, int C) { return g_nt[kind] < 0 ? npix * C * 2 >= NT_MIN_BYTES : g_nt[kind] != 0; }
#else
inline bool nt_pass(int, long long npix, int C) { return npix * C * 2 >= NT_MIN_BYTES; }
#endif
template <bool NTL>
__device__ __forceinline__ bf16x8 ld8(const __bf16 *p) {
    if constexpr (NTL) return __builtin_nontemporal_load((const bf16x8 *)p);
    else return *(const bf16x8 *)p;
}
template <bool NTL>
__device__ __forceinline__ void st8(__bf16 *p, const bf16x8 &v) {
    if constexpr (NTL) __builtin_nontemporal_store(v, (bf16x8 *)p);
    else *(bf16x8 *)p = v;
}

template <int ACT, bool NTL = false>
__global__ void bn_act_fwd_kernel(const __bf16 *__restrict__ z, int z_cs, const float *__restrict__ scale,
                                  const float *__restrict__ shift, const float *__restrict__ slope_p,
                                  const __bf16 *__restrict__ res, int res_cs, __bf16 *__restrict__ y, int y_cs,
                                  long long npix, int C) {
    const int cpr = C / 8;
    const long long total = npix * cpr;
    const float slope = slope_p ? slope_p[0] : 0.f;
    for (long long i = (long long)blockIdx.x * blockDim.x + threadIdx.x; i < total;
         i += (long long)gridDim.x * blockDim.x) {
        const long long pix = i / cpr;
        const int c = (int)(i % cpr) * 8;
        const bf16x8 v = ld8<NTL>(z + pix * z_cs + c);
        bf16x8 o;
#pragma unroll
        for (int e = 0; e < 8; e++) {
            float u = (float)v[e] * scale[c + e] + shift[c + e];
            if (ACT == 1) u = u > 0.f ? u : u * slope;
            else if (ACT == 2) u = mish_f(u);
            o[e] = (__bf16)u;
        }
        if (res) {
            const bf16x8 r = ld8<NTL>(res + pix * res_cs + c);
#pragma unroll
            for (int e = 0; e < 8; e++) o[e] = (__bf16)((float)o[e] + (float)r[e]);
        }
        st8<NTL>(y + pix * y_cs + c, o);
    }
}

constexpr int BWD_SLAB_MIN = 128;
#ifdef RYOLO_MP_ABLATION
static int g_bwd_slabs = 1024, g_bwd_slab_min = BWD_SLAB_MIN;
inline long long bwd_slab(long long npix) {
    long long s = (npix + g_bwd_slabs - 1) / g_bwd_slabs;
    return s < g_bwd_slab_min ? g_bwd_slab_min : s;
}
#else
inline long long bwd_slab(long long npix) {
    const long long s = (npix + 1023) / 1024;
    return s < BWD_SLAB_MIN ? BWD_SLAB_MIN : s;
}
#endif
template <int ACT, bool NTL = false>
__global__ void __launch_bounds__(256)
bn_act_bwd_reduce_kernel(const __bf16 *__restrict__ z, int z_cs, const __bf16 *__restrict__ dy, int dy_cs,
                         const float *__restrict__ scale, const float *__restrict__ shift,
                         const float *__restrict__ mean, const float *__restrict__ invstd,
                         const float *__restrict__ slope_p, long long npix, int C, int CT, float *__restrict__ part, long long SL) {
    __shared__ float red[256][25];
    const int cl = threadIdx.x % CT, pl = threadIdx.x / CT, npl = 256 / CT;
    const int c = (blockIdx.x * CT + cl) * 8;
    const int slab = blockIdx.y;
    const long long p0 = (long long)slab * SL;
    const long long p1 = p0 + SL < npix ? p0 + SL : npix;
    const float slope = slope_p ? slope_p[0] : 0.f;
    float s1[8], s2[8], s3[8];
#pragma unroll
    for (int e = 0; e < 8; e++) s1[e] = s2[e] = s3[e] = 0.f;
    if (c < C) {
        float sc[8], sh[8], mu[8], is[8];
#pragma unroll
        for (int e = 0; e < 8; e++) {
            sc[e] = scale ? scale[c + e] : 1.f; sh[e] = scale ? shift[c + e] : 0.f;
            mu[e] = scale ? mean[c + e] : 0.f; is[e] = scale ? invstd[c + e] : 0.f;
        }
        auto accum = [&](const bf16x8 &zv, const bf16x8 &gv) {
#pragma unroll
            for (int e = 0; e < 8; e++) {
                const float zf = (float)zv[e], d = (float)gv[e];
                float g = d;
                if (scale) {
                    const float u = zf * sc[e] + sh[e];
                    if (ACT == 1 && u <= 0.f) { g = d * slope; s3[e] += d * u; }
                    else if (ACT == 2) g = d * mish_grad(u);
                    s2[e] += g * (zf - mu[e]);
                }
                s1[e] += g;
            }
        };
        long long pix = p0 + pl;
        for (; pix + 3 * npl < p1; pix += 4 * npl) {
            bf16x8 zv[4], gv[4];
#pragma unroll
            for (int k = 0; k < 4; k++) {
                zv[k] = ld8<NTL>(z + (pix + k * npl) * z_cs + c);
                gv[k] = ld8<NTL>(dy + (pix + k * npl) * dy_cs + c);
            }
#pragma unroll
            for (int k = 0; k < 4; k++) accum(zv[k], gv[k]);
        }
        for (; pix < p1; pix += npl) accum(*(const bf16x8 *)(z + pix * z_cs + c), *(const bf16x8 *)(dy + pix * dy_cs + c));
#pragma unroll
        for (int e = 0; e < 8; e++) s2[e] *= is[e];
    }
#pragma unroll
    for (int e = 0; e < 8; e++) { red[threadIdx.x][e] = s1[e]; red[threadIdx.x][8 + e] = s2[e]; red[threadIdx.x][16 + e] = s3[e]; }
    __syncthreads();
    for (int t = threadIdx.x; t < CT * 24; t += 256) {
        const int l = t / 24, k = t % 24;
        float v = 0.f;
        for (int q = 0; q < npl; q++) v += red[q * CT + l][k];
        const int ch = (blockIdx.x * CT + l) * 8 + (k & 7);
        if (ch < C) part[((size_t)slab * 3 + (k >> 3)) * C + ch] = v;
    }
}

__global__ void __launch_bounds__(1024)
bn_act_bwd_finalize_kernel(const float *__restrict__ part, int nslab, int C, float *__restrict__ s1o,
                           float *__restrict__ s2o, float *__restrict__ dgamma, float *__restrict__ dbeta,
                           float *__restrict__ s3o) {
    __shared__ float red[3][32][33];
    const int cx = threadIdx.x & 31, ry = threadIdx.x >> 5;
    const int c = blockIdx.x * 32 + cx;
    float a = 0.f, b = 0.f, d = 0.f;
    if (c < C) {
        for (int s0 = ry; s0 < nslab; s0 += 32 * 8) {
            float va[8], vb[8], vd[8];
#pragma unroll
            for (int u = 0; u < 8; u++) {
                const int s = s0 + 32 * u;
                va[u] = s < nslab ? part[((size_t)s * 3 + 0) * C + c] : 0.f;
                vb[u] = s < nslab ? part[((size_t)s * 3 + 1) * C + c] : 0.f;
                vd[u] = s < nslab ? part[((size_t)s * 3 + 2) * C + c] : 0.f;
            }
#pragma unroll
            for (int u = 0; u < 8; u++) { a += va[u]; b += vb[u]; d += vd[u]; }
        }
    }
    red[0][ry][cx] = a; red[1][ry][cx] = b; red[2][ry][cx] = d;
    __syncthreads();
    if (ry != 0) return;
    for (int k = 1; k < 32; k++) { a += red[0][k][cx]; b += red[1][k][cx]; d += red[2][k][cx]; }
    if (c < C) {
        s1o[c] = a;
        s2o[c] = b;
        if (dgamma) dgamma[c] += b;
        if (dbeta) dbeta[c] += a;
        if (s3o) s3o[c] = d;
    }
}

constexpr int BWD_FOLD = 64, BWD_FOLD_MIN_ROWS = 2048;
__global__ void __launch_bounds__(1024)
bn_act_bwd_fold_kernel(const float *__restrict__ part, int nrows, int C, int per, float *__restrict__ out) {
// ... 461 lines not shown
#ifdef RYOLO_MP_ABLATION
#define RYOLO_WG_ABL(A) if (w.T == 256 && g_wgrad_abl == A) { hipFuncSetAttribute((const void *)wgrad_wide_kernel<256, 128, A>, hipFuncAttributeMaxDynamicSharedMemorySize, WIDE_LDS); hipLaunchKernelGGL((wgrad_wide_kernel<256, 128, A>), dim3(nblk), dim3(256), WIDE_LDS, stream, p); } else
        RYOLO_WG_ABL(1) RYOLO_WG_ABL(2) RYOLO_WG_ABL(4) RYOLO_WG_ABL(6) RYOLO_WG_ABL(7)
#undef RYOLO_WG_ABL
        if (w.T == 261) {
            constexpr int LDS261 = 3 * 32 * (256 + 256) * 2;
            hipFuncSetAttribute((const void *)wgrad_wide_kernel<256, 256, 0, 8>, hipFuncAttributeMaxDynamicSharedMemorySize, LDS261);
            hipLaunchKernelGGL((wgrad_wide_kernel<256, 256, 0, 8>), dim3(nblk), dim3(512), LDS261, stream, p);
        } else if (w.T == 256 && g_wgrad_abl == 8) {
            hipFuncSetAttribute((const void *)wgrad_wide_kernel<256, 128, 0, 8>, hipFuncAttributeMaxDynamicSharedMemorySize, WIDE_LDS);
            hipLaunchKernelGGL((wgrad_wide_kernel<256, 128, 0, 8>), dim3(nblk), dim3(512), WIDE_LDS, stream, p);
        } else if (w.T == 263) {
            hipLaunchKernelGGL((wgrad_wide_kernel<128, 64>), dim3(nblk), dim3(256), 3 * 32 * (128 + 64) * 2, stream, p);
        } else
#endif
        if (w.T == 256) hipLaunchKernelGGL((wgrad_wide_kernel<256, 128>), dim3(nblk), dim3(256), WIDE_LDS, stream, p);
        else if (w.T == 258) hipLaunchKernelGGL((wgrad_wide_kernel<128, 64, 0, 4, 3>), dim3(nblk), dim3(256), 3 * 32 * (128 + 3 * 64) * 2, stream, p);
        else if (w.T == 259) hipLaunchKernelGGL((wgrad_wide_kernel<128, 128>), dim3(nblk), dim3(256), 3 * 32 * (128 + 128) * 2, stream, p);
        else if (w.T == 260) hipLaunchKernelGGL((wgrad_wide_kernel<64, 128>), dim3(nblk), dim3(256), 3 * 32 * (64 + 128) * 2, stream, p);
        else hipLaunchKernelGGL((wgrad_wide_kernel<128, 256>), dim3(nblk), dim3(256), WIDE_LDS, stream, p);
    } else if (w.T == 128) hipLaunchKernelGGL(wgrad_kernel<128>, dim3(nblk), dim3(256), 2 * 2 * KP * 128 * 2, stream, p);
    else if (w.T == 64) hipLaunchKernelGGL(wgrad_kernel<64>, dim3(nblk), dim3(256), 2 * 2 * KP * 64 * 2, stream, p);
    else hipLaunchKernelGGL(wgrad_kernel<32>, dim3(nblk), dim3(256), 2 * 2 * KP * 32 * 2, stream, p);
    if (hipGetLastError() != hipSuccess) return RYOLO_ELAUNCH;
    if (do_reduce) launch_wgrad_reduce((const float *)workspace, w.S, d->Cout, Cin_real, d->Cin, d->ksize, p.Kpad, p.Cout_pad, grad_oihw, accumulate, stream);
    return ok_launch();
}

int ryolo_bn_finalize(double *stat_part, int rows, int cpad, int C, long long count, float eps, float momentum,
                      const float *gamma, const float *beta, float *mean, float *invstd, float *scale, float *shift,
                      float *running_mean, float *running_var, void *stream) {
    if (!stat_part || !gamma || !beta || !mean || !invstd || !scale || !shift || rows <= 0 || C <= 0 || count <= 0)
        return RYOLO_EINVAL;
    hipLaunchKernelGGL(bn_finalize_kernel, dim3((C + 31) / 32), dim3(1024), 0, (hipStream_t)stream, stat_part, rows, cpad, C,
                       (float)count, eps, momentum, gamma, beta, mean, invstd, scale, shift, running_mean, running_var);
    return ok_launch();
}

int ryolo_bn_act_fwd(const void *z, int z_cstride, const float *scale, const float *shift, int act, const float *slope,
                     const void *residual, int res_cstride, void *y, int y_cstride, long long npix, int C, void *stream) {
    if (!z || !scale || !shift || !y || npix <= 0 || C <= 0 || (C & 7) || (z_cstride & 7) || (y_cstride & 7))
        return RYOLO_EINVAL;
    if (act < 0 || act > 2) return RYOLO_EINVAL;
    const bool ntl = nt_pass(0, npix, C);
#define RYOLO_BN_FWD(A)                                                                                                   \
    hipLaunchKernelGGL((ntl ? bn_act_fwd_kernel<A, true> : bn_act_fwd_kernel<A, false>), dim3(grid_for(npix * (C / 8))), dim3(256), 0, (hipStream_t)stream,           \
                       (const __bf16 *)z, z_cstride, scale, shift, slope, (const __bf16 *)residual, res_cstride,          \
                       (__bf16 *)y, y_cstride, npix, C)
    if (act == 0) RYOLO_BN_FWD(0); else if (act == 1) RYOLO_BN_FWD(1); else RYOLO_BN_FWD(2);
#undef RYOLO_BN_FWD
    return ok_launch();
}

size_t ryolo_bn_act_bwd_workspace_bytes(long long npix, int C) {
    const long long nslab = (npix + bwd_slab(npix) - 1) / bwd_slab(npix);
    return (size_t)nslab * 3 * C * 4 + (size_t)3 * C * 4;
}

static int bn_act_bwd_impl(const void *z, int z_cstride, const void *dy, int dy_cstride, const float *scale, const float *shift,
                           const float *mean, const float *invstd, int act, const float *slope, void *dz, int dz_cstride,
                           long long npix, int C, float *dgamma, float *dbeta, float *dslope, void *workspace,
                           size_t workspace_bytes, const float *pre_part, int pre_rows, void *stream_);

int ryolo_bn_act_bwd(const void *z, int z_cstride, const void *dy, int dy_cstride, const float *scale, const float *shift,
                     const float *mean, const float *invstd, int act, const float *slope, void *dz, int dz_cstride,
                     long long npix, int C, float *dgamma, float *dbeta, float *dslope, void *workspace,
                     size_t workspace_bytes, void *stream_) {
    return bn_act_bwd_impl(z, z_cstride, dy, dy_cstride, scale, shift, mean, invstd, act, slope, dz, dz_cstride, npix, C, dgamma, dbeta,
                           dslope, workspace, workspace_bytes, nullptr, 0, stream_);
}

int ryolo_bn_act_bwd_reduced(const void *z, int z_cstride, const void *dy, int dy_cstride, const float *scale, const float *shift,
                             const float *mean, const float *invstd, int act, const float *slope, void *dz, int dz_cstride,
                             long long npix, int C, float *dgamma, float *dbeta, float *dslope, const float *part, int rows,
                             void *workspace, size_t workspace_bytes, void *stream_) {
    if (!part || rows <= 0 || !scale || act != 1) return RYOLO_EINVAL;
    return bn_act_bwd_impl(z, z_cstride, dy, dy_cstride, scale, shift, mean, invstd, act, slope, dz, dz_cstride, npix, C, dgamma, dbeta,
                           dslope, workspace, workspace_bytes, part, rows, stream_);
}

static int bn_act_bwd_impl(const void *z, int z_cstride, const void *dy, int dy_cstride, const float *scale, const float *shift,
                           const float *mean, const float *invstd, int act, const float *slope, void *dz, int dz_cstride,
                           long long npix, int C, float *dgamma, float *dbeta, float *dslope, void *workspace,
                           size_t workspace_bytes, const float *pre_part, int pre_rows, void *stream_) {
    if (!z || !dy || npix <= 0 || C <= 0 || (C & 7) || (z_cstride & 7) || (dy_cstride & 7) || !workspace) return RYOLO_EINVAL;
    if (workspace_bytes < (pre_part ? (size_t)3 * C * 4 : ryolo_bn_act_bwd_workspace_bytes(npix, C))) return RYOLO_EINVAL;
    if (scale && (!shift || !mean || !invstd || !dz || (dz_cstride & 7))) return RYOLO_EINVAL;
    hipStream_t stream = (hipStream_t)stream_;
    int nslab = pre_part ? pre_rows : (int)((npix + bwd_slab(npix) - 1) / bwd_slab(npix));
    float *part = pre_part ? const_cast<float *>(pre_part) : (float *)workspace;
    float *s1 = pre_part ? (float *)workspace : part + (size_t)nslab * 3 * C, *s2 = s1 + C, *s3 = s2 + C;
    if (pre_part && pre_rows >= BWD_FOLD_MIN_ROWS && workspace_bytes >= (size_t)(3 + 3 * BWD_FOLD) * C * 4) {
        float *folded = s3 + C;
        const int per = (pre_rows + BWD_FOLD - 1) / BWD_FOLD;
        hipLaunchKernelGGL(bn_act_bwd_fold_kernel, dim3((C + 31) / 32, BWD_FOLD), dim3(1024), 0, stream, part, pre_rows, C, per, folded);
        part = folded;
        nslab = (pre_rows + per - 1) / per;
    }
    float *dsl = (scale && act == 1) ? dslope : nullptr;
    int CT = 32;
    while (CT > 1 && CT > C / 8) CT >>= 1;
    if (act < 0 || act > 2) return RYOLO_EINVAL;
    const bool nt_red = nt_pass(1, npix, C), nt_app = nt_pass(2, npix, C);
#define RYOLO_BN_REDK(A) (nt_red ? bn_act_bwd_reduce_kernel<A, true> : bn_act_bwd_reduce_kernel<A, false>)
#define RYOLO_BN_RED(A)                                                                                                   \
    hipLaunchKernelGGL(RYOLO_BN_REDK(A), dim3((C / 8 + CT - 1) / CT, nslab), dim3(256), 0, stream,             \
                       (const __bf16 *)z, z_cstride, (const __bf16 *)dy, dy_cstride, scale, shift, mean, invstd, slope,   \
                       npix, C, CT, part, bwd_slab(npix))
    if (pre_part) {  }
    else if (act == 0) RYOLO_BN_RED(0); else if (act == 1) RYOLO_BN_RED(1); else RYOLO_BN_RED(2);
#undef RYOLO_BN_RED
    hipLaunchKernelGGL(bn_act_bwd_finalize_kernel, dim3((C + 31) / 32), dim3(1024), 0, stream, part, nslab, C, s1, s2,
                       scale ? dgamma : nullptr, dbeta, dsl ? s3 : nullptr);
#define RYOLO_BN_APP(A)                                                                                                   \
    hipLaunchKernelGGL((nt_app ? bn_act_bwd_apply_kernel<A, true> : bn_act_bwd_apply_kernel<A, false>), dim3(grid_for(npix * (C / 8), 256, ELEM_BLOCKS)), dim3(256), 0, stream,                  \
                       (const __bf16 *)z, z_cstride, (const __bf16 *)dy, dy_cstride, scale, shift, mean, invstd, s1, s2,  \
                       1.0f / (float)npix, slope, (__bf16 *)dz, dz_cstride, npix, C, s3, dsl)
    if (scale) {
        if (act == 0) RYOLO_BN_APP(0); else if (act == 1) RYOLO_BN_APP(1); else RYOLO_BN_APP(2);
    }
#undef RYOLO_BN_APP
    return ok_launch();
}

#ifdef RYOLO_MP_ABLATION
void ryolo_debug_bn_set(int slabs, int slab_min, int nt_fwd, int nt_red, int nt_app) {
    g_bwd_slabs = slabs; g_bwd_slab_min = slab_min; g_nt[0] = nt_fwd; g_nt[1] = nt_red; g_nt[2] = nt_app;
}
#endif

int ryolo_upsample2x_bwd(const void *dy, int dy_cstride, void *dx, int dx_cstride, int N, int H, int W, int C,
                         int accumulate, void *stream) {
    if (!dy || !dx || N <= 0 || H <= 0 || W <= 0 || C <= 0 || (C & 7) || (dy_cstride & 7) || (dx_cstride & 7))
        return RYOLO_EINVAL;
    hipLaunchKernelGGL(upsample2x_bwd_kernel, dim3(grid_for((long long)N * H * W * (C / 8))), dim3(256), 0,
                       (hipStream_t)stream, (const __bf16 *)dy, dy_cstride, (__bf16 *)dx, dx_cstride, N, H, W, C, accumulate);
    return ok_launch();
}

int ryolo_pgrad_to_nhwc(const float *pgrad, int bs, int na, int ny, int nx, int no, void *out, int out_cstride,
                        void *stream) {
    if (!pgrad || !out || bs <= 0 || na <= 0 || ny <= 0 || nx <= 0 || no <= 0 || out_cstride < na * no) return RYOLO_EINVAL;
    const long long npix = (long long)bs * ny * nx;
    const size_t smem = (size_t)PG_PIX * na * no * 2;
    if ((na * no) % 8 == 0 && (out_cstride & 7) == 0 && (((uintptr_t)out) & 15) == 0 && smem <= 64 * 1024 && npix < 0x7fffffffll) {
        hipLaunchKernelGGL(pgrad_to_nhwc_tiled_kernel, dim3((unsigned)((npix + PG_PIX - 1) / PG_PIX)), dim3(256), smem,
                           (hipStream_t)stream, pgrad, na, ny * nx, no, (__bf16 *)out, out_cstride, (int)npix);
        return ok_launch();
    }
    hipLaunchKernelGGL(pgrad_to_nhwc_kernel, dim3(grid_for((long long)bs * na * ny * nx * no)), dim3(256), 0,
                       (hipStream_t)stream, pgrad, bs, na, ny, nx, no, (__bf16 *)out, out_cstride);
    return ok_launch();
}

}
```

### rotate-yolov3_amd/model/hip_train_ops.py

```python
import ctypes as C

import torch

from .. import _lib
from .hip_ops import ConvDesc, _check_nhwc, cpad

_vp = C.c_void_p
_P = C.POINTER(ConvDesc)
_lib.declare("ryolo_conv_stat_rows", C.c_int, [_P])
_lib.declare("ryolo_conv2d_bn_act_stats", C.c_int, [_P, _vp, _vp, _vp, _vp, _vp, _vp, _vp, _vp])
_lib.declare("ryolo_bn_finalize", C.c_int, [_vp, C.c_int, C.c_int, C.c_int, C.c_longlong, C.c_float, C.c_float, _vp, _vp, _vp,
                                            _vp, _vp, _vp, _vp, _vp, _vp])
_lib.declare("ryolo_bn_act_fwd", C.c_int, [_vp, C.c_int, _vp, _vp, C.c_int, _vp, _vp, C.c_int, _vp, C.c_int, C.c_longlong,
                                           C.c_int, _vp])
_lib.declare("ryolo_bn_act_bwd_workspace_bytes", C.c_size_t, [C.c_longlong, C.c_int])
_lib.declare("ryolo_bn_act_bwd", C.c_int, [_vp, C.c_int, _vp, C.c_int, _vp, _vp, _vp, _vp, C.c_int, _vp, _vp, C.c_int,
                                           C.c_longlong, C.c_int, _vp, _vp, _vp, _vp, C.c_size_t, _vp])
_lib.declare("ryolo_conv_packed_dgrad_bytes", C.c_size_t, [C.c_int, C.c_int, C.c_int, C.c_int])
_lib.declare("ryolo_conv_pack_weights_dgrad", C.c_int, [_vp, C.c_int, C.c_int, C.c_int, C.c_int, _vp, _vp, _vp])
_lib.declare("ryolo_conv_dgrad_tap_table", C.c_int, [C.c_int, C.c_int, _vp])
_lib.declare("ryolo_conv2d_dgrad", C.c_int, [_P, _vp, C.c_int, _vp, _vp, _vp, _vp, C.c_int, _vp])
_lib.declare("ryolo_conv2d_dgrad_bnreduce", C.c_int, [_P, _vp, C.c_int, _vp, _vp, _vp, _vp, C.c_int, _vp, C.c_int, _vp, _vp, _vp, _vp, _vp,
                                                      _vp, _vp])
_lib.declare("ryolo_bn_act_bwd_reduced", C.c_int, [_vp, C.c_int, _vp, C.c_int, _vp, _vp, _vp, _vp, C.c_int, _vp, _vp, C.c_int,
                                                   C.c_longlong, C.c_int, _vp, _vp, _vp, _vp, C.c_int, _vp, C.c_size_t, _vp])
_lib.declare("ryolo_conv_wgrad_workspace_bytes", C.c_size_t, [_P])
_lib.declare("ryolo_conv2d_wgrad", C.c_int, [_P, _vp, _vp, C.c_int, C.c_int, _vp, C.c_int, _vp, C.c_size_t, _vp])
_lib.declare("ryolo_conv2d_wgrad_partials", C.c_int, [_P, _vp, _vp, C.c_int, C.c_int, _vp, C.c_int, _vp, C.c_size_t, _vp])
_lib.declare("ryolo_conv2d_wgrad_reduce", C.c_int, [_P, _vp, _vp, C.c_int, C.c_int, _vp, C.c_int, _vp, C.c_size_t, _vp])
_lib.declare("ryolo_upsample2x_bwd", C.c_int, [_vp, C.c_int, _vp, C.c_int, C.c_int, C.c_int, C.c_int, C.c_int, C.c_int, _vp])
_lib.declare("ryolo_pgrad_to_nhwc", C.c_int, [_vp, C.c_int, C.c_int, C.c_int, C.c_int, C.c_int, _vp, C.c_int, _vp])


_lib.declare("ryolo_yolo_loss_bitmap_bytes", C.c_size_t, [C.c_longlong])
_lib.declare("ryolo_yolo_loss", C.c_int, [_vp, C.c_int, C.c_int, C.c_int, C.c_int, C.c_int, C.c_int, _vp, C.c_int, _vp, _vp, _vp,
                                          _vp, _vp, _vp, _vp, _vp, _vp, C.c_float, C.c_float, C.c_float, C.c_float, C.c_float,
                                          C.c_float, C.c_int, _vp, _vp, _vp, _vp])
_lib.declare("ryolo_yolo_loss_nhwc", C.c_int, [_vp, C.c_int, _vp, C.c_int, C.c_int, C.c_int, C.c_int, C.c_int, C.c_int, _vp, C.c_int, _vp,
                                               _vp, _vp, _vp, _vp, _vp, _vp, _vp, _vp, C.c_float, C.c_float, C.c_float, C.c_float,
                                               C.c_float, C.c_float, C.c_int, _vp, _vp, _vp, C.c_int, _vp, _vp])
_lib.declare("ryolo_scale_bf16_if", C.c_int, [_vp, _vp, C.c_int, C.c_longlong, C.c_int, _vp])
_lib.declare("ryolo_yolo_loss_bitmap_bytes_arc", C.c_size_t, [C.c_longlong, C.c_int, C.c_int])
_lib.declare("ryolo_yolo_loss_arc", C.c_int, [_vp] + [C.c_int] * 6 + [_vp, C.c_int] + [_vp] * 9 + [C.c_float] * 6 +
             [C.c_int, C.c_int, C.c_float] + [_vp] * 4)
_lib.declare("ryolo_yolo_loss_nhwc_arc", C.c_int, [_vp, C.c_int, _vp] + [C.c_int] * 6 + [_vp, C.c_int] + [_vp] * 9 + [C.c_float] * 6 +
             [C.c_int, C.c_int, C.c_float] + [_vp, _vp, _vp, C.c_int, _vp, _vp])
ARC_FOCAL, ARC_UBCE, ARC_UCE = 1, 2, 4


def arc_flags(arc):
    f = ARC_FOCAL if 'F' in arc else 0
    if 'default' in arc:
        return f
    if 'BCE' in arc:
        return f | ARC_UBCE
    if 'CE' in arc:
        return f | ARC_UCE
    raise ValueError("unknown arc %r" % (arc,))
_lib.declare("ryolo_riou_loss_pairs", C.c_int, [_vp, _vp, C.c_int, _vp, _vp, _vp])


class PackJob(C.Structure):
    _fields_ = [("src", C.c_void_p), ("dst", C.c_void_p), ("kind", C.c_int), ("Cout", C.c_int), ("Cin", C.c_int),
# ... 51 lines not shown

    def __init__(self, device):
        self.device = device
        self.jobs = []

    def add(self, weight, stride, cin_pad, packed_fwd, packed_dgrad):
        cout, cin, k, _ = weight.shape
        tmp = (PackJob * 8)()
        n = _lib.lib().ryolo_conv_pack_job_fill(tmp, weight.data_ptr(), cout, cin, k, stride, cin_pad, packed_fwd.data_ptr(),
                                                packed_dgrad.data_ptr() if packed_dgrad is not None else None)
        if n <= 0:
            raise RuntimeError("ryolo_conv_pack_job_fill failed")
        for q in range(n):
            j = PackJob()
            C.memmove(C.byref(j), C.byref(tmp[q]), C.sizeof(PackJob))
            self.jobs.append(j)

    def finalize(self):
        arr = (PackJob * len(self.jobs))()
        blk = 0
        for q, j in enumerate(self.jobs):
            nb = j.block_end
            j.block_begin, j.block_end = blk, blk + nb
            blk += nb
            arr[q] = j
        self.total_blocks = blk
        raw = bytes(arr)
        self.dev_jobs = torch.frombuffer(bytearray(raw), dtype=torch.uint8).to(self.device)
        self.n = len(self.jobs)

    def run(self):
        _lib.check(_lib.lib().ryolo_conv_pack_batch(self.dev_jobs.data_ptr(), self.n, self.total_blocks, _s(self.device)),
                   "ryolo_conv_pack_batch")


def _s(dev):
    return _lib.stream_ptr(dev)


def make_desc(x, cout, ksize, stride, pad, out_cs=None, tile=0):
    in_cs = _check_nhwc(x, "x")
    n, h, w, cin = x.shape
    return ConvDesc(n, h, w, cin, cout, ksize, stride, pad, in_cs, out_cs or cout, 0, 0, 0.0, 1, tile)


def stat_rows():
    d = ConvDesc(1, 8, 8, 8, 8, 1, 1, 0, 8, 8, 0, 0, 0.0, 1, 0)
    rows = _lib.lib().ryolo_conv_stat_rows(C.byref(d))
    if rows <= 0:
        raise RuntimeError("ryolo_conv_stat_rows failed")
    return rows


def conv_fwd_stats(d, x, packed_w, ones, shift, z, part=None, clear=True):
    L = _lib.lib()
    rows = L.ryolo_conv_stat_rows(C.byref(d))
    cp = cpad(d.Cout)
    if part is None:
        part = torch.zeros((rows, 2, cp), dtype=torch.float64, device=x.device)
    else:
        part = part.view(-1)[:rows * 2 * cp].view(rows, 2, cp)
        if clear:
            part.zero_()
    if z is not None:
        d.out_cstride = _check_nhwc(z, "z")
    _lib.check(L.ryolo_conv2d_bn_act_stats(C.byref(d), x.data_ptr(), packed_w.data_ptr(), ones.data_ptr(), shift.data_ptr(),
                                           None, z.data_ptr() if z is not None else None, part.data_ptr(), _s(x.device)),
               "ryolo_conv2d_bn_act_stats")
    return part


_lib.declare("ryolo_conv0_bn_act_fwd", C.c_int, [C.POINTER(ConvDesc), _vp, _vp, _vp, _vp, C.c_int, _vp, _vp, _vp])
_lib.declare("ryolo_conv0_bn_bwd_workspace_bytes", C.c_size_t, [])
_lib.declare("ryolo_conv0_bn_bwd", C.c_int, [C.POINTER(ConvDesc), _vp, _vp, _vp, C.c_int, _vp, _vp, _vp, _vp, C.c_int, _vp, _vp, C.c_int,
                                             _vp, _vp, _vp, _vp, C.c_size_t, C.c_int, _vp])


def conv0_recompute_supported(d):
    return bool(_lib.lib().ryolo_conv0_recompute_supported(C.byref(d)))


def conv0_bn_act_fwd(d, x, packed_w, scale, shift, act, slope, y):
    d.out_cstride = _check_nhwc(y, "y")
    _lib.check(_lib.lib().ryolo_conv0_bn_act_fwd(C.byref(d), x.data_ptr(), packed_w.data_ptr(), scale.data_ptr(), shift.data_ptr(), act,
                                                 slope.data_ptr() if slope is not None else None, y.data_ptr(), _s(x.device)),
               "ryolo_conv0_bn_act_fwd")
    return y


def conv0_bn_bwd_ws(device):
    return torch.zeros(_lib.lib().ryolo_conv0_bn_bwd_workspace_bytes(), dtype=torch.uint8, device=device)


def conv0_bn_bwd(d, x, packed_w, dy, stats, act, slope, dz, dgamma, dbeta, dslope, ws, ws_is_zero=True):
    mean, invstd, scale, shift = stats
    _lib.check(_lib.lib().ryolo_conv0_bn_bwd(C.byref(d), x.data_ptr(), packed_w.data_ptr(), dy.data_ptr(), dy.stride(2),
                                             scale.data_ptr(), shift.data_ptr(), mean.data_ptr(), invstd.data_ptr(), act,
                                             slope.data_ptr() if slope is not None else None, dz.data_ptr(), dz.stride(2),
                                             dgamma.data_ptr(), dbeta.data_ptr(), dslope.data_ptr() if dslope is not None else None,
                                             ws.data_ptr(), ws.numel(), 1 if ws_is_zero else 0, _s(x.device)), "ryolo_conv0_bn_bwd")
    return dz


_lib.declare("ryolo_conv0_bn_bwd_wgrad_workspace_bytes", C.c_size_t, [])
_lib.declare("ryolo_conv0_bn_bwd_wgrad", C.c_int, [C.POINTER(ConvDesc), _vp, _vp, _vp, C.c_int, _vp, _vp, _vp, _vp, C.c_int, _vp, _vp, _vp, _vp,
                                                  _vp, C.c_int, C.c_int, _vp, C.c_size_t, _vp])


def conv0_bn_bwd_wgrad_ws(device):
    return torch.empty(_lib.lib().ryolo_conv0_bn_bwd_wgrad_workspace_bytes(), dtype=torch.uint8, device=device)


def conv0_bn_bwd_wgrad(d, x, packed_w, dy, stats, act, slope, dgamma, dbeta, dslope, grad_w, cin_real, accumulate, ws):
    mean, invstd, scale, shift = stats
    _lib.check(_lib.lib().ryolo_conv0_bn_bwd_wgrad(C.byref(d), x.data_ptr(), packed_w.data_ptr(), dy.data_ptr(), dy.stride(2),
                                                   scale.data_ptr(), shift.data_ptr(), mean.data_ptr(), invstd.data_ptr(), act,
                                                   slope.data_ptr() if slope is not None else None, dgamma.data_ptr(), dbeta.data_ptr(),
                                                   dslope.data_ptr() if dslope is not None else None, grad_w.data_ptr(), int(cin_real),
                                                   1 if accumulate else 0, ws.data_ptr(), ws.numel(), _s(x.device)), "ryolo_conv0_bn_bwd_wgrad")


def conv_fwd_plain(d, x, packed_w, ones, shift, z):
    d.out_cstride = _check_nhwc(z, "z")
    _lib.check(_lib.lib().ryolo_conv2d_bn_act(C.byref(d), x.data_ptr(), packed_w.data_ptr(), ones.data_ptr(), shift.data_ptr(),
                                              None, z.data_ptr(), _s(x.device)), "ryolo_conv2d_bn_act")


def bn_finalize(part, C_, count, gamma, beta, eps=1e-5, momentum=0.1, running_mean=None, running_var=None, out=None):
    dev = part.device
    if out is None:
        out = [torch.empty(C_, dtype=torch.float32, device=dev) for _ in range(4)]
    _lib.check(_lib.lib().ryolo_bn_finalize(part.data_ptr(), part.shape[0], part.shape[2], C_, int(count), eps, momentum,
                                            gamma.data_ptr(), beta.data_ptr(), out[0].data_ptr(), out[1].data_ptr(),
                                            out[2].data_ptr(), out[3].data_ptr(),
                                            running_mean.data_ptr() if running_mean is not None else None,
                                            running_var.data_ptr() if running_var is not None else None, _s(dev)),
               "ryolo_bn_finalize")
    return out


def bn_act_fwd(z, scale, shift, act, slope, y, residual=None):
    n, h, w, c = z.shape
    _lib.check(_lib.lib().ryolo_bn_act_fwd(z.data_ptr(), z.stride(2), scale.data_ptr(), shift.data_ptr(), act,
                                           slope.data_ptr() if slope is not None else None,
                                           residual.data_ptr() if residual is not None else None,
                                           residual.stride(2) if residual is not None else 0, y.data_ptr(), y.stride(2),
                                           n * h * w, c, _s(z.device)), "ryolo_bn_act_fwd")
    return y


def bn_act_bwd(z, dy, stats, act, slope, dz, dgamma, dbeta, dslope, ws):
    n, h, w, c = z.shape
    mean, invstd, scale, shift = stats if stats is not None else (None, None, None, None)
    p = lambda t: t.data_ptr() if t is not None else None
    _lib.check(_lib.lib().ryolo_bn_act_bwd(z.data_ptr(), z.stride(2), dy.data_ptr(), dy.stride(2), p(scale), p(shift), p(mean),
                                           p(invstd), act, p(slope), p(dz), dz.stride(2) if dz is not None else 0,
                                           n * h * w, c, p(dgamma), p(dbeta), p(dslope), ws.data_ptr(), ws.numel(),
                                           _s(z.device)), "ryolo_bn_act_bwd")


def bn_bwd_ws_bytes(npix, c):
    return _lib.lib().ryolo_bn_act_bwd_workspace_bytes(npix, c)


_tap_tables = {}


def dgrad_tap_table(ksize, stride, device):
    key = (ksize, stride, device.index)
    t = _tap_tables.get(key)
    if t is None:
        host = (C.c_int * 72)()
        _lib.check(_lib.lib().ryolo_conv_dgrad_tap_table(ksize, stride, host), "ryolo_conv_dgrad_tap_table")
        t = torch.tensor(list(host), dtype=torch.int32, device=device)
        _tap_tables[key] = t
    return t


def pack_weights_dgrad(weight, stride, out=None):
    cout, cin, k, _ = weight.shape
    L = _lib.lib()
    nbytes = L.ryolo_conv_packed_dgrad_bytes(cout, cin, k, stride)
    if out is None:
        out = torch.empty(nbytes, dtype=torch.uint8, device=weight.device)
    w = weight.contiguous()
    table = dgrad_tap_table(k, stride, weight.device)
    _lib.check(L.ryolo_conv_pack_weights_dgrad(w.data_ptr(), cout, cin, k, stride, out.data_ptr(), table.data_ptr(),
                                               _s(weight.device)), "ryolo_conv_pack_weights_dgrad")
    return out


def conv_dgrad(d, dz, packed_dgrad, ones, zeros, dx, accumulate):
    _lib.check(_lib.lib().ryolo_conv2d_dgrad(C.byref(d), dz.data_ptr(), dz.stride(2), packed_dgrad.data_ptr(), ones.data_ptr(),
                                             zeros.data_ptr(), dx.data_ptr(), 1 if accumulate else 0, _s(dz.device)),
               "ryolo_conv2d_dgrad")


def dgrad_bnreduce_rows(d):
    return _lib.lib().ryolo_conv2d_dgrad_bnreduce_rows(C.byref(d))


def conv_dgrad_bnreduce(d, dz, packed_dgrad, ones, zeros, dx, accumulate, z, stats, slope, part):
    mean, invstd, scale, shift = stats
    _lib.check(_lib.lib().ryolo_conv2d_dgrad_bnreduce(C.byref(d), dz.data_ptr(), dz.stride(2), packed_dgrad.data_ptr(), ones.data_ptr(),
                                                      zeros.data_ptr(), dx.data_ptr(), 1 if accumulate else 0, z.data_ptr(), z.stride(2),
                                                      scale.data_ptr(), shift.data_ptr(), mean.data_ptr(), invstd.data_ptr(),
                                                      slope.data_ptr(), part.data_ptr(), _s(dz.device)), "ryolo_conv2d_dgrad_bnreduce")

# ... 145 lines not shown
```

### rotate-yolov3_amd/model/plan.py

```python
import ctypes as C
from collections import namedtuple

from .. import _lib
from .._lib import ACT_LINEAR, ConvDesc

View = namedtuple('View', 'buf off C H W cs')
EvalPlan = namedtuple('EvalPlan', 'shapes buffers x views ops')
TrainPlan = namedtuple('TrainPlan', 'shapes buffers x act grd forward blocks backward')


class Refused(RuntimeError):
    """the configuration is refused at plan time (as opposed to a bug in the planner)"""


def _abs(i, l):
    return l if l > 0 else i + l


def _sources(i, d):
    return [_abs(i, int(v)) for v in d['layers'].split(',')]


def _new(buffers, c, h, w):
    buffers.append((c, h, w))
# ... 258 lines not shown
        elif t == 'shortcut':
            a, b = i - 1, _abs(i, int(d['from']))
            act[i], grd[i] = pair_for(i)
            forward.append(('add', i, (act[a], act[b], act[i], grd[a], grd[b], grd[i])))
        elif t == 'upsample':
            act[i], grd[i] = pair_for(i)
            forward.append(('up', i, (act[i - 1], act[i], grd[i - 1], grd[i])))
        elif t == 'route':
            if i in alias:
                act[i], grd[i] = act[alias[i]], grd[alias[i]]
        elif t == 'yolo':
            act[i], grd[i] = act[i - 1], grd[i - 1]
            forward.append(('yolo', i, (act[i], grd[i])))

    init = set()

    def first(g):
        if g in init:
            return False
        init.add(g)
        init.update(children.get(g, ()))
        return True

    heads = [i for kind, i, _ in forward if kind == 'yolo']
    backward = []
    for kind, i, pl in reversed(forward):
        if kind == 'yolo':
            first(pl[1])
            backward.append((kind, i, heads.index(i)))
        elif kind == 'conv':
            res_first = first(pl['res_g']) if (pl['res_g'] is not None and not pl['res_alias']) else None
            backward.append((kind, i, (res_first, first(pl['xin_g']) if pl['xin_g'] is not None else None)))
        elif kind == 'add':
            backward.append((kind, i, (first(pl[3]), first(pl[4]))))
        elif kind == 'up':
            backward.append((kind, i, first(pl[2])))
    return TrainPlan(shp, buffers, x, act, grd, forward, blocks, backward)


def reduce_fusion_pairs(tp):
    by = {b['layer']: b for b in tp.blocks}
    pairs = []
    for (k0, i0, _), (k1, i1, _) in zip(tp.backward[:-1], tp.backward[1:]):
        if k0 != 'conv' or k1 != 'conv':
            continue
        x, y = by[i0], by[i1]
        g, dy = x['xin_g'], y['dy']
        if g is None or not y['bn'] or y['recompute'] or g != dy or dy[2:5] != y['shape'] or g.cs != g.C:
            continue
        rows = _query('ryolo_conv2d_dgrad_bnreduce_rows', x['desc'])
        if rows > 0:
            pairs.append((x, y, rows))
    return pairs
```

### rotate-yolov3_amd/model/train_engine.py

```python
import ctypes as C
import os

import torch
import torch.nn as nn

from .. import _lib
from . import hip_ops as ops
from . import hip_train_ops as tr
from . import plan
from .engine import HipEngine


class _Fn(torch.autograd.Function):
    @staticmethod
    def forward(ctx, engine, x, anchor):
        ctx.engine = engine
        outs = engine.forward(x)
        return tuple(outs)

    @staticmethod
    def backward(ctx, *grads):
        ctx.engine.backward(grads)
        return None, None, None


class TrainEngine(object):
    def __init__(self, model, x_shape, device, use_graph=True):
        _lib.lib()
        self.model = model
        self.no_graph_env = os.environ.get('RYOLO_NO_GRAPH', '0') == '1'
        self.use_graph = use_graph and not self.no_graph_env
        self.graph_fallback = None
        self.reduce_fallback = None
        self.force_eager = False
        self.g_fwd = self.g_bwd = None
        self._segs = None
        self._red_planned = False
        self.nbt = None
        self.packs = None
        self.steps = 0
        self.device = device
        self.bs, cin, self.H, self.W = [int(v) for v in x_shape]
        defs, mods = model.module_defs, model.module_list
        self.defs, self.mods = defs, mods

        convs = {i: self._conv_attrs(mods[i]) for i, d in enumerate(defs) if d['type'] == 'convolutional'}
        tp = self._tplan = plan.plan_train(defs, convs, self.bs, self.H, self.W,
                                           conv0_recompute=os.environ.get('RYOLO_CONV0_RECOMPUTE', '1') != '0',
                                           conv0_one_pass=os.environ.get('RYOLO_CONV0_ONE_PASS', '1') != '0', cin=cin)
        self.shp = tp.shapes

        def new_buf(c, h, w):
            return torch.empty((self.bs, h, w, c), dtype=torch.bfloat16, device=device)

        bufs = [new_buf(*b) for b in tp.buffers]
        tensors = {None: None}

        def tv(v):
            if v not in tensors:
                tensors[v] = bufs[v.buf][..., v.off:v.off + v.C]
            return tensors[v]

        self.x_nhwc = tv(tp.x)
        cmax = max(ops.cpad(max(c.out_channels, c.in_channels)) for c in (HipEngine._conv_of(mods[i]) for i in convs))
        self.ones = torch.ones(cmax, device=device)
        self.zeros = torch.zeros(cmax, device=device)
        self.stat_part = torch.zeros((tr.stat_rows(), 2, cmax), dtype=torch.float64, device=device)
        self.blocks = []
        self.p, self.p_src = [], []
        self.static_grad = {}
        self.direct = False
        self.static_flat = None
        wgrad_ws, bn_ws = 0, 0
        self.plan = fwd = []
        for kind, i, rec in tp.forward:
            if kind == 'conv':
                conv = HipEngine._conv_of(mods[i])
                bn = HipEngine._bn_of(mods[i])
                actmod = [s_ for s_ in mods[i] if isinstance(s_, (nn.PReLU, nn.LeakyReLU))]
                xin, y, dy = tv(rec['xin']), tv(rec['y']), tv(rec['dy'])
                c, h, w = rec['shape']
                desc = ops.ConvDesc(*rec['desc'])
                if bn is not None:
                    z = None if rec['recompute'] else new_buf(c, h, w)
                    dz = None if rec['one_pass'] else new_buf(c, h, w)
                else:
                    z, dz = y, dy
                blk = dict(i=i, conv=conv, bn=bn, act=actmod[-1] if actmod else None, mish=any(type(s_).__name__ == 'Mish' for s_ in mods[i]),
                           xin=xin, xin_g=tv(rec['xin_g']), z=z, dz=dz, y=y, dy=dy, desc=desc, res=tv(rec['res']), res_g=tv(rec['res_g']),
                           res_alias=rec['res_alias'], cin_k=xin.shape[-1], k=desc.ksize, s=desc.stride, pad=desc.pad,
                           npix=self.bs * h * w, C=c, recompute=rec['recompute'])
                wgrad_ws = max(wgrad_ws, tr.wgrad_ws_bytes(desc))
                bn_ws = max(bn_ws, tr.bn_bwd_ws_bytes(blk['npix'], c))
                self.blocks.append(blk)
                fwd.append(('conv', i, blk))
            elif kind in ('add', 'up'):
                fwd.append((kind, i, tuple(tv(v) for v in rec)))
            elif kind == 'yolo':
                m = mods[i]
                c, h, w = tp.shapes[i]
                anchors = m.anchors.to(device=device, dtype=torch.float32).contiguous()
                pbuf = torch.empty((self.bs, m.na, h, w, model.nc + 6), dtype=torch.float32, device=device)
                io = None
                if model.nc + 6 > 96 or m.na * (model.nc + 6) > 1024:
                    io = torch.empty((self.bs, m.na * h * w, model.nc + 6), dtype=torch.float32, device=device)
                self.p.append(pbuf)
                fwd.append(('yolo', i, (tv(rec[0]), tv(rec[1]), m, anchors, pbuf, io, h, w)))
        self.head_pairs = [(pl[0], pl[1]) for kind, _, pl in fwd if kind == 'yolo']
        self.fused_nhwc = False
        self.head_g_ready = False
        self.batch_reduce = os.environ.get('RYOLO_WGRAD_BATCH_REDUCE', '1') != '0'
        self._wr_batches = {}
        self._ws_w_bytes = max(wgrad_ws, 256)
        self._ws_w = None
        self.ws_b = torch.empty(max(bn_ws, 256), dtype=torch.uint8, device=device)

        self.bplan = [(kind, i, pl, flags) for (kind, i, pl), (_, _, flags) in zip(reversed(fwd), tp.backward)]

    @staticmethod
    def _conv_attrs(m):
# ... 157 lines not shown
            _lib.check(_lib.lib().ryolo_nchw_f32_to_nhwc_bf16(x.data_ptr(), n, c, h, w, 8, self.x_nhwc.data_ptr(), _lib.stream_ptr(dev)),
                       "ryolo_nchw_f32_to_nhwc_bf16")
            if not self.use_graph or self.steps < 2 or self.force_eager:
                self._forward_launch()
            else:
                if self.g_fwd is None:
                    self.g_fwd = self._capture(self._forward_launch)
                if self.g_fwd is not None:
                    self.g_fwd.replay()
        return [p for p in self.p]

    def _capture(self, launch):
        dev = self.device
        torch.cuda.synchronize(dev)
        g = torch.cuda.CUDAGraph()
        try:
            with torch.cuda.graph(g, capture_error_mode="thread_local"):
                launch()
            return g
        except Exception as e:
            self.use_graph = False
            self.graph_fallback = "%s: %s" % (type(e).__name__, str(e).splitlines()[0][:200] if str(e) else "")
            import warnings
            warnings.warn("TrainEngine: hipGraph capture failed (%s); continuing with eager launches" % self.graph_fallback)
            try:
                torch.cuda.synchronize(dev)
            except Exception:
                pass
            launch()
            return None

    def _forward_launch(self):
        dev = self.device
        L = _lib.lib()
        if self.nbt is None:
            self.nbt = [pl['bn'].num_batches_tracked for kind, i, pl in self.plan if kind == 'conv' and pl['bn'] is not None]
        if self.nbt:
            torch._foreach_add_(self.nbt, 1)
        if self.packs is None:
            self.packs = tr.WeightPackBatch(dev)
            for kind, i, pl in self.plan:
                if kind != 'conv':
                    continue
                w = pl['conv'].weight
                if w.dtype != torch.float32 or not w.is_contiguous():
                    raise RuntimeError("TrainEngine expects contiguous fp32 conv weights")
                cout, cin, k, _ = w.shape
                pl['packed'] = torch.empty(L.ryolo_conv_packed_weight_bytes(cout, pl['cin_k'], k), dtype=torch.uint8, device=dev)
                pl['packed_d'] = torch.empty(L.ryolo_conv_packed_dgrad_bytes(cout, cin, k, pl['s']), dtype=torch.uint8,
                                             device=dev) if pl['xin_g'] is not None else None
                self.packs.add(w.detach(), pl['s'], pl['cin_k'], pl['packed'], pl['packed_d'])
            self.packs.finalize()
        self.packs.run()
        for kind, i, pl in self.plan:
            if kind == 'conv':
                b = pl
                conv, bn = b['conv'], b['bn']
                if bn is not None:
                    part = tr.conv_fwd_stats(b['desc'], b['xin'], b['packed'], self.ones, self.zeros, b['z'], part=self.stat_part,
                                             clear=False)
                    b['stats'] = tr.bn_finalize(part, b['C'], b['npix'], bn.weight.detach(), bn.bias.detach(), eps=bn.eps,
                                                momentum=bn.momentum, running_mean=bn.running_mean,
                                                running_var=bn.running_var, out=b.get('stats'))
                    slope = b['act'].weight.detach() if isinstance(b['act'], nn.PReLU) else None
                    if isinstance(b['act'], nn.LeakyReLU):
                        if 'leaky' not in b:
                            b['leaky'] = torch.full((1,), b['act'].negative_slope, device=dev)
                        slope = b['leaky']
                    b['slope'] = slope
                    b['actcode'] = 2 if b['mish'] else (1 if slope is not None else 0)
                    if b['recompute']:
                        tr.conv0_bn_act_fwd(b['desc'], b['xin'], b['packed'], b['stats'][2], b['stats'][3], b['actcode'], slope, b['y'])
                    else:
                        tr.bn_act_fwd(b['z'], b['stats'][2], b['stats'][3], b['actcode'], slope, b['y'], residual=b['res'])
                else:
                    if conv.bias is not None:
                        if 'bias_pad' not in b:
                            b['bias_pad'] = torch.zeros(ops.cpad(b['C']), device=dev)
                        b['bias_pad'][:b['C']].copy_(conv.bias.detach())
                        bias = b['bias_pad']
                    else:
                        bias = self.zeros
                    tr.conv_fwd_plain(b['desc'], b['xin'], b['packed'], self.ones, bias, b['z'])
                    b['stats'] = None
            elif kind == 'add':
                a, bb, y = pl[0], pl[1], pl[2]
                nn_, hh, ww, cc = y.shape
                _lib.check(L.ryolo_add_nhwc(a.data_ptr(), a.stride(2), bb.data_ptr(), bb.stride(2), y.data_ptr(), y.stride(2),
                                            nn_ * hh * ww, cc, _lib.stream_ptr(dev)), "ryolo_add_nhwc")
            elif kind == 'up':
                xin, y = pl[0], pl[1]
                nn_, hh, ww, cc = xin.shape
                _lib.check(L.ryolo_upsample_nhwc(xin.data_ptr(), xin.stride(2), y.data_ptr(), y.stride(2), nn_, hh, ww, cc, 2,
                                                 _lib.stream_ptr(dev)), "ryolo_upsample_nhwc")
            elif kind == 'yolo':
                head, _, m, anchors, pbuf, io, hh, ww = pl
                stride = float(max(self.H, self.W)) / float(max(hh, ww))
                _lib.check(L.ryolo_yolo_decode(head.data_ptr(), head.stride(2), self.bs, hh, ww, m.na, self.model.nc + 6,
                                               anchors.data_ptr(), stride, 1.0, 0, io.data_ptr() if io is not None else None, m.na * hh * ww, 0,
                                               pbuf.data_ptr(), _lib.stream_ptr(dev)), "ryolo_yolo_decode")
                if (m.nx, m.ny) != (ww, hh):
                    from .models import create_grids
                    create_grids(m, (self.H, self.W), (ww, hh), dev)

    def backward(self, pgrads):
        dev = self.device
        with torch.cuda.device(dev), torch.no_grad():
            if not hasattr(self, "static_pg"):
                self.static_pg = [torch.zeros_like(p) for p in self.p]
            ready = self.head_g_ready
            self.head_g_ready = False
# ... 130 lines not shown
```

Baseline: 1369 images/s.

## Fuse BN finalize into BN-act forward and shrink stat partial rows

Adds a kernel that reduces the per-row BN statistic partials, computes per-channel scale/shift and running stats, then applies normalize+activation(+residual) in the same launch. This replaces the separate bn_finalize launch for non-recompute BN convs. Conv kernels now take a runtime row mask, so these layers write only 8 partial rows into a pre-zeroed per-layer scratch, which keeps the per-block reduction cheap. The trade-off is more atomic contention on fewer rows, and every pixel-slab block redundantly recomputes the channel stats.

```diff
diff --git a/include/ryolo.h b/include/ryolo.h
--- a/include/ryolo.h
+++ b/include/ryolo.h
@@ -125,12 +125,19 @@
                               const float *shift, const void *residual, void *y,
                               double *stat_part ,
                               void *stream);
+int ryolo_conv2d_bn_act_stats_nr(const ryolo_conv_desc *desc, const void *x, const void *w_packed, const float *scale,
+                                 const float *shift, const void *residual, void *y, double *stat_part, int stat_rows, void *stream);
 int ryolo_bn_finalize(double *stat_part, int rows, int cpad, int C, long long count, float eps, float momentum,
                       const float *gamma, const float *beta, float *mean, float *invstd, float *scale, float *shift,
                       float *running_mean , float *running_var, void *stream);
 int ryolo_bn_act_fwd(const void *z, int z_cstride, const float *scale, const float *shift, int act,
                      const float *slope , const void *residual, int res_cstride, void *y,
                      int y_cstride, long long npix, int C, void *stream);
+int ryolo_bn_stats_act_fwd(const double *stat_part, int rows, int cpad, long long count, float eps, float momentum, const float *gamma,
+                           const float *beta, float *mean, float *invstd, float *scale, float *shift,
+                           float *running_mean , float *running_var, const void *z, int z_cstride, int act,
+                           const float *slope , const void *residual, int res_cstride, void *y,
+                           int y_cstride, long long npix, int C, int chunk, void *stream);
 size_t ryolo_bn_act_bwd_workspace_bytes(long long npix, int C);
 int ryolo_bn_act_bwd(const void *z, int z_cstride, const void *dy, int dy_cstride, const float *scale, const float *shift,
                      const float *mean, const float *invstd, int act, const float *slope, void *dz, int dz_cstride,
diff --git a/rotate-yolov3_amd/csrc/conv.hip b/rotate-yolov3_amd/csrc/conv.hip
--- a/rotate-yolov3_amd/csrc/conv.hip
+++ b/rotate-yolov3_amd/csrc/conv.hip
@@ -345,7 +345,7 @@
             for (int w = 1; w < WGM; w++) v += slot[w * 2 * BN + tid];
             const int st = tid / BN, ch = tid % BN;
             if (n0 + ch < p.Cout)
-                atomicAdd(p.stat_part + (size_t)(m_tile % STAT_ROWS) * 2 * p.stat_cpad + (size_t)st * p.stat_cpad + n0 + ch, (double)v);
+                atomicAdd(p.stat_part + (size_t)(m_tile & p.stat_rmask) * 2 * p.stat_cpad + (size_t)st * p.stat_cpad + n0 + ch, (double)v);
         }
     }
 
@@ -625,7 +625,7 @@
             for (int w = 1; w < WGM; w++) v += slots[w * 2 * BN + tid];
             const int st = tid / BN, c = tid % BN;
             if (n0 + c < p.Cout)
-                atomicAdd(p.stat_part + ((size_t)(blockIdx.x % STAT_ROWS) * 2 + st) * p.stat_cpad + n0 + c, (double)v);
+                atomicAdd(p.stat_part + ((size_t)(blockIdx.x & p.stat_rmask) * 2 + st) * p.stat_cpad + n0 + c, (double)v);
         }
         __syncthreads();
     };
@@ -1056,7 +1056,7 @@
             }
         if (fr < 8) {
             const int ch = (fr >> 2) * 16 + g * 4 + (fr & 3);
-            double *row = p.stat_part + (size_t)(wave_id % STAT_ROWS) * 2 * p.stat_cpad;
+            double *row = p.stat_part + (size_t)(wave_id & p.stat_rmask) * 2 * p.stat_cpad;
             atomicAdd(row + ch, (double)ta);
             atomicAdd(row + p.stat_cpad + ch, (double)tb);
         }
@@ -1523,7 +1523,13 @@
 
 int ryolo_conv2d_bn_act_stats(const ryolo_conv_desc *d, const void *x, const void *w_packed, const float *scale,
                               const float *shift, const void *residual, void *y, double *stat_part, void *stream_) {
+    return ryolo_conv2d_bn_act_stats_nr(d, x, w_packed, scale, shift, residual, y, stat_part, STAT_ROWS, stream_);
+}
+
+int ryolo_conv2d_bn_act_stats_nr(const ryolo_conv_desc *d, const void *x, const void *w_packed, const float *scale,
+                                   const float *shift, const void *residual, void *y, double *stat_part, int stat_rows, void *stream_) {
     if (validate(d) != RYOLO_OK || !x || !w_packed || !scale || !shift) return RYOLO_EINVAL;
+    if (stat_rows < 1 || stat_rows > STAT_ROWS || (stat_rows & (stat_rows - 1))) return RYOLO_EINVAL;
     if (!y && !(stat_part && ryolo_conv0_recompute_supported(d))) return RYOLO_EINVAL;
     if (residual && ((d->res_cstride & 7) || d->res_cstride < d->Cout)) return RYOLO_EINVAL;
     if (((uintptr_t)x | (uintptr_t)y | (uintptr_t)w_packed | (uintptr_t)residual | (uintptr_t)scale | (uintptr_t)shift) & 15)
@@ -1572,6 +1578,7 @@
     p.nt_out = (long long)p.M * d->upsample * d->upsample * d->Cout * 2 >= nt_out_min_bytes() ? 1 : 0;
     p.stat_part = stat_part;
     p.stat_cpad = (d->Cout + 127) / 128 * 128;
+    p.stat_rmask = stat_rows - 1;
     const unsigned long long c8_xb = (unsigned long long)d->N * d->H * d->W * 16ull, c8_yb = ((unsigned long long)(p.M - 1) * d->out_cstride + 32) * 2ull;
     if (d->ksize == 3 && d->stride == 1 && d->pad == 1 && d->Cin == 8 && d->in_cstride == 8 && d->Cout == 32 &&
         !residual && d->upsample == 1 && !(d->tile & 0x1ff) && p.Wo >= 16 && c8_xb < 0x7fffff00ull && c8_yb < 0x7fffff00ull) {
diff --git a/rotate-yolov3_amd/csrc/conv_common.h b/rotate-yolov3_amd/csrc/conv_common.h
--- a/rotate-yolov3_amd/csrc/conv_common.h
+++ b/rotate-yolov3_amd/csrc/conv_common.h
@@ -50,6 +50,7 @@
     unsigned y_bytes, res_bytes;
     double *stat_part;
     int stat_cpad;
+    int stat_rmask = STAT_ROWS - 1;
     int nt_out;
     int reg3;
     int korder = 0;
diff --git a/rotate-yolov3_amd/csrc/conv_mp.hip b/rotate-yolov3_amd/csrc/conv_mp.hip
--- a/rotate-yolov3_amd/csrc/conv_mp.hip
+++ b/rotate-yolov3_amd/csrc/conv_mp.hip
@@ -457,7 +457,7 @@
                 }
                 stamp_e(3 + h);
                 if (GEN == 1 && p.stat_part) {
-                    double *row = p.stat_part + (size_t)(((m0 / BM) * 2 + wm) % STAT_ROWS) * 2 * p.stat_cpad;
+                    double *row = p.stat_part + (size_t)(((m0 / BM) * 2 + wm) & p.stat_rmask) * 2 * p.stat_cpad;
                     float *slot = stat_lds + ((size_t)((n0 / MP_BN) * 2 + wm) * 2) * MP_BN + wn * 64;
                     float ta = 0.f, tb = 0.f;
 #pragma unroll
@@ -505,7 +505,7 @@
         if (stat_in_lds) {
             asm volatile("s_waitcnt lgkmcnt(0)" ::: "memory");
             __builtin_amdgcn_s_barrier();
-            double *row = p.stat_part + (size_t)(blockIdx.x % STAT_ROWS) * 2 * p.stat_cpad;
+            double *row = p.stat_part + (size_t)(blockIdx.x & p.stat_rmask) * 2 * p.stat_cpad;
             for (int i = tid; i < p.nt * 2 * MP_BN; i += 512) {
                 const int s_ = i / (2 * MP_BN), st = (i / MP_BN) & 1, ch = i % MP_BN;
                 const float *q = stat_lds + ((size_t)(s_ * 2) * 2 + st) * MP_BN + ch;
diff --git a/rotate-yolov3_amd/csrc/conv_mq.hip b/rotate-yolov3_amd/csrc/conv_mq.hip
--- a/rotate-yolov3_amd/csrc/conv_mq.hip
+++ b/rotate-yolov3_amd/csrc/conv_mq.hip
@@ -507,7 +507,7 @@
                     }
                 }
                 if (GEN == 1 && p.stat_part) {
-                    double *row = p.stat_part + (size_t)((m0 / L::BM) % STAT_ROWS) * 2 * p.stat_cpad;
+                    double *row = p.stat_part + (size_t)((m0 / L::BM) & p.stat_rmask) * 2 * p.stat_cpad;
                     float *slot = stat_lds + (size_t)(n0 / Q_BN) * 2 * Q_BN + wn * CW;
                     float ta = 0.f, tb = 0.f;
 #pragma unroll
@@ -553,7 +553,7 @@
         if (stat_in_lds) {
             asm volatile("s_waitcnt lgkmcnt(0)" ::: "memory");
             __builtin_amdgcn_s_barrier();
-            double *row = p.stat_part + (size_t)(blockIdx.x % STAT_ROWS) * 2 * p.stat_cpad;
+            double *row = p.stat_part + (size_t)(blockIdx.x & p.stat_rmask) * 2 * p.stat_cpad;
             for (int i = tid; i < p.nt * 2 * Q_BN; i += 256) {
                 const int s_ = i / (2 * Q_BN), st = (i / Q_BN) & 1, ch = i % Q_BN;
                 const float v = stat_lds[(size_t)(s_ * 2 + st) * Q_BN + ch];
diff --git a/rotate-yolov3_amd/csrc/conv_pw.hip b/rotate-yolov3_amd/csrc/conv_pw.hip
--- a/rotate-yolov3_amd/csrc/conv_pw.hip
+++ b/rotate-yolov3_amd/csrc/conv_pw.hip
@@ -431,7 +431,7 @@
         if (fr < CF * 4) {
             const int ch = n0 + wave * CF * 16 + (fr >> 2) * 16 + g * 4 + (fr & 3);
             if (ch < p.Cout) {
-                double *row = p.stat_part + (size_t)(blockIdx.x % STAT_ROWS) * 2 * p.stat_cpad;
+                double *row = p.stat_part + (size_t)(blockIdx.x & p.stat_rmask) * 2 * p.stat_cpad;
                 atomicAdd(row + ch, (double)ta);
                 atomicAdd(row + p.stat_cpad + ch, (double)tb);
             }
diff --git a/rotate-yolov3_amd/csrc/conv_stem.hip b/rotate-yolov3_amd/csrc/conv_stem.hip
--- a/rotate-yolov3_amd/csrc/conv_stem.hip
+++ b/rotate-yolov3_amd/csrc/conv_stem.hip
@@ -187,7 +187,7 @@
             float v = slots[st * COUT + c];
 #pragma unroll
             for (int w = 1; w < 4; w++) v += slots[(w * 2 + st) * COUT + c];
-            atomicAdd(p.stat_part + ((size_t)(blockIdx.x % STAT_ROWS) * 2 + st) * p.stat_cpad + c, (double)v);
+            atomicAdd(p.stat_part + ((size_t)(blockIdx.x & p.stat_rmask) * 2 + st) * p.stat_cpad + c, (double)v);
         }
     }
 }
@@ -820,7 +820,7 @@
             }
         if (fr < 8) {
             const int ch = co0 + (fr >> 2) * 16 + g * 4 + (fr & 3);
-            double *row = p.stat_part + (size_t)(blockIdx.x % STAT_ROWS) * 2 * p.stat_cpad;
+            double *row = p.stat_part + (size_t)(blockIdx.x & p.stat_rmask) * 2 * p.stat_cpad;
             atomicAdd(row + ch, (double)ta);
             atomicAdd(row + p.stat_cpad + ch, (double)tb);
         }
diff --git a/rotate-yolov3_amd/csrc/rnms.hip b/rotate-yolov3_amd/csrc/rnms.hip
--- a/rotate-yolov3_amd/csrc/rnms.hip
+++ b/rotate-yolov3_amd/csrc/rnms.hip
@@ -849,7 +849,7 @@
     }
 }
 
-int ryolo_abi_version(void) { return 3; }
+int ryolo_abi_version(void) { return 4; }
 
 void ryolo_rnms_count_pairs(uint64_t *device_counter) { g_pair_counter = (unsigned long long *)device_counter; }
 
diff --git a/rotate-yolov3_amd/csrc/train.hip b/rotate-yolov3_amd/csrc/train.hip
--- a/rotate-yolov3_amd/csrc/train.hip
+++ b/rotate-yolov3_amd/csrc/train.hip
@@ -835,6 +835,24 @@
     else wgrad_reduce_body<1>(sm, bid, nblk, j.part, j.S, j.Cout, j.Cin_real, j.Cin_k, j.ks, j.Kpad, j.Cout_pad, j.g, j.accumulate);
 }
 
+struct BnChan { float mean, invstd, scale, shift, run_mean, run_var; };
+__device__ __forceinline__ BnChan bn_channel(double s, double q, float count, float eps, float momentum, float gamma, float beta,
+                                             float run_mean, float run_var) {
+    const double mu = s / count;
+    double var = q / count - mu * mu;
+    if (var < 0) var = 0;
+    const float is = (float)(1.0 / sqrt(var + (double)eps));
+    BnChan o;
+    o.mean = (float)mu;
+    o.invstd = is;
+    o.scale = gamma * is;
+    o.shift = beta - (float)mu * gamma * is;
+    const double unb = count > 1.f ? var * count / (count - 1.0) : var;
+    o.run_mean = (1.f - momentum) * run_mean + momentum * (float)mu;
+    o.run_var = (1.f - momentum) * run_var + momentum * (float)unb;
+    return o;
+}
+
 __global__ void __launch_bounds__(1024) bn_finalize_kernel(double *__restrict__ part, int R, int cpad, int C, float count, float eps,
                                    float momentum, const float *__restrict__ gamma, const float *__restrict__ beta,
                                    float *__restrict__ mean, float *__restrict__ invstd, float *__restrict__ scale,
@@ -869,18 +887,14 @@
     __syncthreads();
     if (ry != 0 || c >= C) return;
     for (int k = 1; k < 32; k++) { s += red[0][k][cx]; q += red[1][k][cx]; }
-    const double mu = s / count;
-    double var = q / count - mu * mu;
-    if (var < 0) var = 0;
-    const float is = (float)(1.0 / sqrt(var + (double)eps));
-    mean[c] = (float)mu;
-    invstd[c] = is;
-    scale[c] = gamma[c] * is;
-    shift[c] = beta[c] - (float)mu * gamma[c] * is;
+    const BnChan o = bn_channel(s, q, count, eps, momentum, gamma[c], beta[c], run_mean ? run_mean[c] : 0.f, run_mean ? run_var[c] : 0.f);
+    mean[c] = o.mean;
+    invstd[c] = o.invstd;
+    scale[c] = o.scale;
+    shift[c] = o.shift;
     if (run_mean) {
-        const double unb = count > 1.f ? var * count / (count - 1.0) : var;
-        run_mean[c] = (1.f - momentum) * run_mean[c] + momentum * (float)mu;
-        run_var[c] = (1.f - momentum) * run_var[c] + momentum * (float)unb;
+        run_mean[c] = o.run_mean;
+        run_var[c] = o.run_var;
     }
 }
 
@@ -944,6 +958,101 @@
     }
 }
 
+constexpr int FOLD_MAX_CL = 32;
+template <int ACT, bool NTL = false>
+__global__ void __launch_bounds__(256)
+bn_stats_act_fwd_kernel(const double *__restrict__ part, int R, int cpad, float count, float eps, float momentum,
+                        const float *__restrict__ gamma, const float *__restrict__ beta, float *__restrict__ mean,
+                        float *__restrict__ invstd, float *__restrict__ scale, float *__restrict__ shift,
+                        float *__restrict__ run_mean, float *__restrict__ run_var, const __bf16 *__restrict__ z, int z_cs,
+                        const float *__restrict__ slope_p, const __bf16 *__restrict__ res, int res_cs, __bf16 *__restrict__ y, int y_cs,
+                        long long npix, int C, int CL, long long PB) {
+    __shared__ float s_sc[FOLD_MAX_CL * 8], s_sh[FOLD_MAX_CL * 8];
+    const int c0 = blockIdx.x * CL * 8;
+    if ((int)threadIdx.x < CL * 8) {
+        const int c = c0 + threadIdx.x;
+        if (c < C) {
+            const double *col = part + c;
+            double s = 0.0, q = 0.0;
+            if (R <= 32) {
+                for (int r0 = 0; r0 < R; r0 += 8) {
+                    double a[8], b[8];
+#pragma unroll
+                    for (int u = 0; u < 8; u++) {
+                        const int r = r0 + u;
+                        a[u] = r < R ? col[(size_t)r * 2 * cpad] : 0.0;
+                        b[u] = r < R ? col[(size_t)r * 2 * cpad + cpad] : 0.0;
+                    }
+#pragma unroll
+                    for (int u = 0; u < 8; u++) { s += a[u]; q += b[u]; }
+                }
+            } else {
+                for (int l = 0; l < 32; l++) {
+                    double a = 0.0, b = 0.0;
+                    for (int r = l; r < R; r += 32) { a += col[(size_t)r * 2 * cpad]; b += col[(size_t)r * 2 * cpad + cpad]; }
+                    if (l == 0) { s = a; q = b; } else { s += a; q += b; }
+                }
+            }
+            const bool first = blockIdx.y == 0;
+            const BnChan o = bn_channel(s, q, count, eps, momentum, gamma[c], beta[c], first && run_mean ? run_mean[c] : 0.f,
+                                        first && run_mean ? run_var[c] : 0.f);
+            s_sc[threadIdx.x] = o.scale;
+            s_sh[threadIdx.x] = o.shift;
+            if (first) {
+                mean[c] = o.mean;
+                invstd[c] = o.invstd;
+                scale[c] = o.scale;
+                shift[c] = o.shift;
+                if (run_mean) {
+                    run_mean[c] = o.run_mean;
+                    run_var[c] = o.run_var;
+                }
+            }
+        }
+    }
+    __syncthreads();
+    const int cl = threadIdx.x % CL, pl = threadIdx.x / CL, npl = 256 / CL;
+    const int c = c0 + cl * 8;
+    if (c >= C) return;
+    float sc[8], sh[8];
+#pragma unroll
+    for (int e = 0; e < 8; e++) { sc[e] = s_sc[cl * 8 + e]; sh[e] = s_sh[cl * 8 + e]; }
+    const float slope = slope_p ? slope_p[0] : 0.f;
+    const long long p0 = (long long)blockIdx.y * PB;
+    const long long p1 = p0 + PB < npix ? p0 + PB : npix;
+    auto one = [&](const bf16x8 &v, const bf16x8 &r, long long pix) {
+        bf16x8 o;
+#pragma unroll
+        for (int e = 0; e < 8; e++) {
+            float u = (float)v[e] * sc[e] + sh[e];
+            if (ACT == 1) u = u > 0.f ? u : u * slope;
+            else if (ACT == 2) u = mish_f(u);
+            o[e] = (__bf16)u;
+        }
+        if (res) {
+#pragma unroll
+            for (int e = 0; e < 8; e++) o[e] = (__bf16)((float)o[e] + (float)r[e]);
+        }
+        st8<NTL>(y + pix * y_cs + c, o);
+    };
+    long long pix = p0 + pl;
+    for (; pix + 3 * npl < p1; pix += 4 * npl) {
+        bf16x8 zv[4], rv[4];
+#pragma unroll
+        for (int k = 0; k < 4; k++) {
+            zv[k] = ld8<NTL>(z + (pix + k * npl) * z_cs + c);
+            if (res) rv[k] = ld8<NTL>(res + (pix + k * npl) * res_cs + c);
+            else rv[k] = zv[k];
+        }
+#pragma unroll
+        for (int k = 0; k < 4; k++) one(zv[k], rv[k], pix + k * npl);
+    }
+    for (; pix < p1; pix += npl) {
+        const bf16x8 zv = ld8<NTL>(z + pix * z_cs + c);
+        one(zv, res ? ld8<NTL>(res + pix * res_cs + c) : zv, pix);
+    }
+}
+
 constexpr int BWD_SLAB_MIN = 128;
 #ifdef RYOLO_MP_ABLATION
 static int g_bwd_slabs = 1024, g_bwd_slab_min = BWD_SLAB_MIN;
@@ -957,7 +1066,7 @@
     return s < BWD_SLAB_MIN ? BWD_SLAB_MIN : s;
 }
 #endif
-template <int ACT, bool NTL = false>
+template <int ACT, bool NTL = false, bool BIAS = false>
 __global__ void __launch_bounds__(256)
 bn_act_bwd_reduce_kernel(const __bf16 *__restrict__ z, int z_cs, const __bf16 *__restrict__ dy, int dy_cs,
                          const float *__restrict__ scale, const float *__restrict__ shift,
@@ -985,7 +1094,7 @@
             for (int e = 0; e < 8; e++) {
                 const float zf = (float)zv[e], d = (float)gv[e];
                 float g = d;
-                if (scale) {
+                if (!BIAS && scale) {
                     const float u = zf * sc[e] + sh[e];
                     if (ACT == 1 && u <= 0.f) { g = d * slope; s3[e] += d * u; }
                     else if (ACT == 2) g = d * mish_grad(u);
@@ -999,13 +1108,18 @@
             bf16x8 zv[4], gv[4];
 #pragma unroll
             for (int k = 0; k < 4; k++) {
-                zv[k] = ld8<NTL>(z + (pix + k * npl) * z_cs + c);
                 gv[k] = ld8<NTL>(dy + (pix + k * npl) * dy_cs + c);
+                if constexpr (BIAS) zv[k] = gv[k];
+                else zv[k] = ld8<NTL>(z + (pix + k * npl) * z_cs + c);
             }
 #pragma unroll
             for (int k = 0; k < 4; k++) accum(zv[k], gv[k]);
         }
-        for (; pix < p1; pix += npl) accum(*(const bf16x8 *)(z + pix * z_cs + c), *(const bf16x8 *)(dy + pix * dy_cs + c));
+        for (; pix < p1; pix += npl) {
+            const bf16x8 gv = ld8<NTL>(dy + pix * dy_cs + c);
+            if constexpr (BIAS) accum(gv, gv);
+            else accum(ld8<NTL>(z + pix * z_cs + c), gv);
+        }
 #pragma unroll
         for (int e = 0; e < 8; e++) s2[e] *= is[e];
     }
@@ -1573,6 +1687,33 @@
     return ok_launch();
 }
 
+int ryolo_bn_stats_act_fwd(const double *stat_part, int rows, int cpad, long long count, float eps, float momentum, const float *gamma,
+                           const float *beta, float *mean, float *invstd, float *scale, float *shift, float *running_mean,
+                           float *running_var, const void *z, int z_cstride, int act, const float *slope, const void *residual,
+                           int res_cstride, void *y, int y_cstride, long long npix, int C, int chunk, void *stream) {
+    if (!stat_part || !gamma || !beta || !mean || !invstd || !scale || !shift || rows <= 0 || count <= 0 || cpad < C) return RYOLO_EINVAL;
+    if (!z || !y || npix <= 0 || C <= 0 || (C & 7) || (z_cstride & 7) || (y_cstride & 7) || (residual && (res_cstride & 7))) return RYOLO_EINVAL;
+    if (act < 0 || act > 2 || (running_mean == nullptr) != (running_var == nullptr)) return RYOLO_EINVAL;
+    if (chunk != 0 && chunk != 32 && chunk != 64 && chunk != 128 && chunk != 256) return RYOLO_EINVAL;
+    int CL = (chunk ? chunk : 64) / 8;
+    while (CL > 1 && CL > C / 8) CL >>= 1;
+    const int nchunk = (C / 8 + CL - 1) / CL, npl = 256 / CL;
+    long long nyb = ELEM_BLOCKS / nchunk < 1 ? 1 : ELEM_BLOCKS / nchunk;
+    long long PB = (npix + nyb - 1) / nyb;
+    PB = (PB + 4 * npl - 1) / (4 * npl) * (4 * npl);
+    nyb = (npix + PB - 1) / PB;
+    if (nyb > 65535) return RYOLO_EINVAL;
+    const bool ntl = nt_pass(0, npix, C);
+#define RYOLO_BN_FOLD(A)                                                                                                  \
+    hipLaunchKernelGGL((ntl ? bn_stats_act_fwd_kernel<A, true> : bn_stats_act_fwd_kernel<A, false>), dim3(nchunk, (unsigned)nyb), dim3(256), 0, \
+                       (hipStream_t)stream, stat_part, rows, cpad, (float)count, eps, momentum, gamma, beta, mean, invstd, scale, shift,        \
+                       running_mean, running_var, (const __bf16 *)z, z_cstride, slope, (const __bf16 *)residual, res_cstride,      \
+                       (__bf16 *)y, y_cstride, npix, C, CL, PB)
+    if (act == 0) RYOLO_BN_FOLD(0); else if (act == 1) RYOLO_BN_FOLD(1); else RYOLO_BN_FOLD(2);
+#undef RYOLO_BN_FOLD
+    return ok_launch();
+}
+
 size_t ryolo_bn_act_bwd_workspace_bytes(long long npix, int C) {
     const long long nslab = (npix + bwd_slab(npix) - 1) / bwd_slab(npix);
     return (size_t)nslab * 3 * C * 4 + (size_t)3 * C * 4;
@@ -1604,7 +1745,8 @@
                            const float *mean, const float *invstd, int act, const float *slope, void *dz, int dz_cstride,
                            long long npix, int C, float *dgamma, float *dbeta, float *dslope, void *workspace,
                            size_t workspace_bytes, const float *pre_part, int pre_rows, void *stream_) {
-    if (!z || !dy || npix <= 0 || C <= 0 || (C & 7) || (z_cstride & 7) || (dy_cstride & 7) || !workspace) return RYOLO_EINVAL;
+    if (!dy || npix <= 0 || C <= 0 || (C & 7) || (dy_cstride & 7) || !workspace) return RYOLO_EINVAL;
+    if (scale ? !z || (z_cstride & 7) : z && (z_cstride & 7)) return RYOLO_EINVAL;
     if (workspace_bytes < (pre_part ? (size_t)3 * C * 4 : ryolo_bn_act_bwd_workspace_bytes(npix, C))) return RYOLO_EINVAL;
     if (scale && (!shift || !mean || !invstd || !dz || (dz_cstride & 7))) return RYOLO_EINVAL;
     hipStream_t stream = (hipStream_t)stream_;
@@ -1629,7 +1771,11 @@
                        (const __bf16 *)z, z_cstride, (const __bf16 *)dy, dy_cstride, scale, shift, mean, invstd, slope,   \
                        npix, C, CT, part, bwd_slab(npix))
     if (pre_part) {  }
-    else if (act == 0) RYOLO_BN_RED(0); else if (act == 1) RYOLO_BN_RED(1); else RYOLO_BN_RED(2);
+    else if (!scale) {
+        hipLaunchKernelGGL((nt_red ? bn_act_bwd_reduce_kernel<0, true, true> : bn_act_bwd_reduce_kernel<0, false, true>),
+                           dim3((C / 8 + CT - 1) / CT, nslab), dim3(256), 0, stream, (const __bf16 *)nullptr, 0, (const __bf16 *)dy, dy_cstride,
+                           scale, shift, mean, invstd, slope, npix, C, CT, part, bwd_slab(npix));
+    } else if (act == 0) RYOLO_BN_RED(0); else if (act == 1) RYOLO_BN_RED(1); else RYOLO_BN_RED(2);
 #undef RYOLO_BN_RED
     hipLaunchKernelGGL(bn_act_bwd_finalize_kernel, dim3((C + 31) / 32), dim3(1024), 0, stream, part, nslab, C, s1, s2,
                        scale ? dgamma : nullptr, dbeta, dsl ? s3 : nullptr);
diff --git a/rotate-yolov3_amd/model/hip_train_ops.py b/rotate-yolov3_amd/model/hip_train_ops.py
--- a/rotate-yolov3_amd/model/hip_train_ops.py
+++ b/rotate-yolov3_amd/model/hip_train_ops.py
@@ -9,6 +9,9 @@
 _P = C.POINTER(ConvDesc)
 _lib.declare("ryolo_conv_stat_rows", C.c_int, [_P])
 _lib.declare("ryolo_conv2d_bn_act_stats", C.c_int, [_P, _vp, _vp, _vp, _vp, _vp, _vp, _vp, _vp])
+_lib.declare("ryolo_conv2d_bn_act_stats_nr", C.c_int, [_P, _vp, _vp, _vp, _vp, _vp, _vp, _vp, C.c_int, _vp])
+_lib.declare("ryolo_bn_stats_act_fwd", C.c_int, [_vp, C.c_int, C.c_int, C.c_longlong, C.c_float, C.c_float] + [_vp] * 9 +
+             [C.c_int, C.c_int, _vp, _vp, C.c_int, _vp, C.c_int, C.c_longlong, C.c_int, C.c_int, _vp])
 _lib.declare("ryolo_bn_finalize", C.c_int, [_vp, C.c_int, C.c_int, C.c_int, C.c_longlong, C.c_float, C.c_float, _vp, _vp, _vp,
                                             _vp, _vp, _vp, _vp, _vp, _vp])
 _lib.declare("ryolo_bn_act_fwd", C.c_int, [_vp, C.c_int, _vp, _vp, C.c_int, _vp, _vp, C.c_int, _vp, C.c_int, C.c_longlong,
@@ -166,9 +169,10 @@
     return rows
 
 
-def conv_fwd_stats(d, x, packed_w, ones, shift, z, part=None, clear=True):
+def conv_fwd_stats(d, x, packed_w, ones, shift, z, part=None, clear=True, rows=None):
     L = _lib.lib()
-    rows = L.ryolo_conv_stat_rows(C.byref(d))
+    lib_rows = L.ryolo_conv_stat_rows(C.byref(d))
+    rows = lib_rows if rows is None else int(rows)
     cp = cpad(d.Cout)
     if part is None:
         part = torch.zeros((rows, 2, cp), dtype=torch.float64, device=x.device)
@@ -178,6 +182,11 @@
             part.zero_()
     if z is not None:
         d.out_cstride = _check_nhwc(z, "z")
+    if rows != lib_rows:
+        _lib.check(L.ryolo_conv2d_bn_act_stats_nr(C.byref(d), x.data_ptr(), packed_w.data_ptr(), ones.data_ptr(), shift.data_ptr(),
+                                                  None, z.data_ptr() if z is not None else None, part.data_ptr(), rows, _s(x.device)),
+                   "ryolo_conv2d_bn_act_stats_nr")
+        return part
     _lib.check(L.ryolo_conv2d_bn_act_stats(C.byref(d), x.data_ptr(), packed_w.data_ptr(), ones.data_ptr(), shift.data_ptr(),
                                            None, z.data_ptr() if z is not None else None, part.data_ptr(), _s(x.device)),
                "ryolo_conv2d_bn_act_stats")
@@ -263,11 +272,29 @@
     return y
 
 
+def bn_stats_act_fwd(part, count, gamma, beta, z, act, slope, y, residual=None, eps=1e-5, momentum=0.1, running_mean=None,
+                     running_var=None, out=None, chunk=0):
+    n, h, w, c = z.shape
+    dev = z.device
+    if out is None:
+        out = [torch.empty(c, dtype=torch.float32, device=dev) for _ in range(4)]
+    _lib.check(_lib.lib().ryolo_bn_stats_act_fwd(part.data_ptr(), part.shape[0], part.shape[2], int(count), eps, momentum,
+                                                 gamma.data_ptr(), beta.data_ptr(), out[0].data_ptr(), out[1].data_ptr(),
+                                                 out[2].data_ptr(), out[3].data_ptr(),
+                                                 running_mean.data_ptr() if running_mean is not None else None,
+                                                 running_var.data_ptr() if running_var is not None else None,
+                                                 z.data_ptr(), z.stride(2), act, slope.data_ptr() if slope is not None else None,
+                                                 residual.data_ptr() if residual is not None else None,
+                                                 residual.stride(2) if residual is not None else 0, y.data_ptr(), y.stride(2),
+                                                 n * h * w, c, int(chunk), _s(dev)), "ryolo_bn_stats_act_fwd")
+    return out
+
+
 def bn_act_bwd(z, dy, stats, act, slope, dz, dgamma, dbeta, dslope, ws):
     n, h, w, c = z.shape
     mean, invstd, scale, shift = stats if stats is not None else (None, None, None, None)
     p = lambda t: t.data_ptr() if t is not None else None
-    _lib.check(_lib.lib().ryolo_bn_act_bwd(z.data_ptr(), z.stride(2), dy.data_ptr(), dy.stride(2), p(scale), p(shift), p(mean),
+    _lib.check(_lib.lib().ryolo_bn_act_bwd(p(z), z.stride(2), dy.data_ptr(), dy.stride(2), p(scale), p(shift), p(mean),
                                            p(invstd), act, p(slope), p(dz), dz.stride(2) if dz is not None else 0,
                                            n * h * w, c, p(dgamma), p(dbeta), p(dslope), ws.data_ptr(), ws.numel(),
                                            _s(z.device)), "ryolo_bn_act_bwd")
diff --git a/rotate-yolov3_amd/model/plan.py b/rotate-yolov3_amd/model/plan.py
--- a/rotate-yolov3_amd/model/plan.py
+++ b/rotate-yolov3_amd/model/plan.py
@@ -334,3 +334,10 @@
         if rows > 0:
             pairs.append((x, y, rows))
     return pairs
+
+
+BN_FOLD_ROWS = 8
+
+
+def bn_fwd_fold(has_bn, recompute):
+    return bool(has_bn) and not recompute
diff --git a/rotate-yolov3_amd/model/train_engine.py b/rotate-yolov3_amd/model/train_engine.py
--- a/rotate-yolov3_amd/model/train_engine.py
+++ b/rotate-yolov3_amd/model/train_engine.py
@@ -66,6 +66,9 @@
         self.ones = torch.ones(cmax, device=device)
         self.zeros = torch.zeros(cmax, device=device)
         self.stat_part = torch.zeros((tr.stat_rows(), 2, cmax), dtype=torch.float64, device=device)
+        self.bn_fold = os.environ.get('RYOLO_BN_FWD_FOLD', '1') != '0'
+        self.fold_rows = plan.BN_FOLD_ROWS
+        self.fold_scratch = None
         self.blocks = []
         self.p, self.p_src = [], []
         self.static_grad = {}
@@ -329,11 +332,34 @@
                 self.packs.add(w.detach(), pl['s'], pl['cin_k'], pl['packed'], pl['packed_d'])
             self.packs.finalize()
         self.packs.run()
+        if self.bn_fold:
+            if self.fold_scratch is None:
+                folded = [pl for kind, i, pl in self.plan if kind == 'conv' and plan.bn_fwd_fold(pl['bn'] is not None, pl['recompute'])]
+                sizes = [self.fold_rows * 2 * ops.cpad(pl['C']) for pl in folded]
+                self.fold_scratch = torch.zeros(max(1, sum(sizes)), dtype=torch.float64, device=dev)
+                off = 0
+                for pl, sz in zip(folded, sizes):
+                    pl['fold_part'] = self.fold_scratch[off:off + sz].view(self.fold_rows, 2, ops.cpad(pl['C']))
+                    off += sz
+            self.fold_scratch.zero_()
         for kind, i, pl in self.plan:
             if kind == 'conv':
                 b = pl
                 conv, bn = b['conv'], b['bn']
-                if bn is not None:
+                if bn is not None and b.get('fold_part') is not None and self.bn_fold:
+                    part = tr.conv_fwd_stats(b['desc'], b['xin'], b['packed'], self.ones, self.zeros, b['z'], part=b['fold_part'],
+                                             clear=False, rows=self.fold_rows)
+                    slope = b['act'].weight.detach() if isinstance(b['act'], nn.PReLU) else None
+                    if isinstance(b['act'], nn.LeakyReLU):
+                        if 'leaky' not in b:
+                            b['leaky'] = torch.full((1,), b['act'].negative_slope, device=dev)
+                        slope = b['leaky']
+                    b['slope'] = slope
+                    b['actcode'] = 2 if b['mish'] else (1 if slope is not None else 0)
+                    b['stats'] = tr.bn_stats_act_fwd(part, b['npix'], bn.weight.detach(), bn.bias.detach(), b['z'], b['actcode'], slope,
+                                                     b['y'], residual=b['res'], eps=bn.eps, momentum=bn.momentum,
+                                                     running_mean=bn.running_mean, running_var=bn.running_var, out=b.get('stats'))
+                elif bn is not None:
                     part = tr.conv_fwd_stats(b['desc'], b['xin'], b['packed'], self.ones, self.zeros, b['z'], part=self.stat_part,
                                              clear=False)
                     b['stats'] = tr.bn_finalize(part, b['C'], b['npix'], bn.weight.detach(), bn.bias.detach(), eps=bn.eps,
```

After: 1357 images/s. Within noise of the previous version (-0.9%).
